# OSU-Nowlab/MPI4DL

Measured on NVIDIA B200. Metric: images/sec (device-timed, max over ranks) AmoebaNet-D 8192^2 hot path (spatial-stage conv/pool fwd+bwd), higher is better.
Workload: dtype bf16

## Files before the change

mpi4dl_b200/csrc/conv_tap.cu:

```cuda
#include <stdlib.h>

#include "common.cuh"
#include "tc_common.cuh"

namespace spc {

using namespace tc;

int make_tmap_ex(CUtensorMap* m, const void* base, int rank, const uint64_t* dims, const uint64_t* strides_bytes,
                 const uint32_t* box, int swizzle128);
int tc_sm_count();

namespace {

constexpr int TAP_THREADS = 448;
constexpr int BLK = 8192;
constexpr int RAW_SHIFT_ROW = 160;
constexpr int MAXRING = 8;
constexpr int STAGE_BYTES = 128 * 128;

struct TapParams {
  int M, Cin, H, W, N;
  int R, ph;
  int Mpad;
  int mrows;
  int a_blk;
  int kchunks;
  int cbox;
  int raw_blk;
  int tiles_w, tiles_h, num_tiles;
  int a_resident, ast, ops;
  int rawb;
  int opblk;
  int group;
  int rows_raw;
  int dbg;
  const __nv_bfloat16* bias;
  __nv_bfloat16* y;
};

struct RingState {
  int s = 0, ph = 0;
  __device__ __forceinline__ void next(int n) { if (++s == n) { s = 0; ph ^= 1; } }
};

template <int D>
__device__ __forceinline__ uint4 shift_window(const uint32_t (&w)[8]) {
  static_assert(D >= -4 && D <= 4, "shift range");
  constexpr int e0 = 4 + D;
  constexpr int k = e0 >> 1;
  uint4 o;
  if (e0 & 1) {
    o.x = __funnelshift_r(w[k], w[k + 1], 16);
    o.y = __funnelshift_r(w[k + 1], w[k + 2], 16);
    o.z = __funnelshift_r(w[k + 2], w[k + 3], 16);
    o.w = __funnelshift_r(w[k + 3], w[k + 4], 16);
  } else {
    o.x = w[k]; o.y = w[k + 1]; o.z = w[k + 2]; o.w = w[k + 3];
  }
  return o;
}

constexpr int SHIFT_THREADS = 256;

template <int NB, int S, int SI>
struct ShiftRow {
  static __device__ __forceinline__ void stores(const uint32_t (&win)[2 * NB][8], int cv, int tid, uint8_t* op_base, int opblk,
                                                int group, uint64_t* op_full, uint64_t* op_empty, RingState& ro, int ops) {
    if constexpr (SI < S) {
      const int q = tid & 7, c0 = tid >> 3;
      const int tile_bytes = NB * opblk;
      if (!group || SI == 0) mbar_wait(&op_empty[ro.s], ro.ph ^ 1);
      uint8_t* opb = op_base + ro.s * (group ? S : 1) * tile_bytes + (group ? SI * tile_bytes : 0);
#pragma unroll
      for (int i = 0; i < 2 * NB; ++i) {
        const int j = i >> 1, c = c0 + 32 * (i & 1);
        if (c < cv)
          *reinterpret_cast<uint4*>(opb + j * opblk + c * 128 + ((q ^ (c & 7)) << 4)) = shift_window<SI - S / 2>(win[i]);
      }
      if (!group || SI == S - 1) {
        fence_proxy_async();
        mbar_arrive(&op_full[ro.s]);
        ro.next(ops);
      }
      ShiftRow<NB, S, SI + 1>::stores(win, cv, tid, op_base, opblk, group, op_full, op_empty, ro, ops);
    }
  }
  static __device__ __forceinline__ void run(const uint8_t* rawr, int raw_blk, int cv, int tid, uint8_t* op_base, int opblk,
                                             int group, uint64_t* op_full, uint64_t* op_empty, RingState& ro, int ops) {
    static_assert(S / 2 <= 4, "filter width <= 9");
    const int q = tid & 7, c0 = tid >> 3;
    uint32_t win[2 * NB][8];
#pragma unroll
    for (int i = 0; i < 2 * NB; ++i) {
      const int j = i >> 1, c = c0 + 32 * (i & 1);
      if (c < cv) {
        const uint8_t* row = rawr + j * raw_blk + c * RAW_SHIFT_ROW;
        const uint4 own = *reinterpret_cast<const uint4*>(row + 16 * (q + 1));
        uint32_t lz = __shfl_up_sync(0xffffffffu, own.z, 1), lw = __shfl_up_sync(0xffffffffu, own.w, 1);
        uint32_t rx = __shfl_down_sync(0xffffffffu, own.x, 1), ry = __shfl_down_sync(0xffffffffu, own.y, 1);
        if (q == 0) { const uint2 h = *reinterpret_cast<const uint2*>(row + 8); lz = h.x; lw = h.y; }
        if (q == 7) { const uint2 h = *reinterpret_cast<const uint2*>(row + 16 * 9); rx = h.x; ry = h.y; }
        win[i][0] = lz; win[i][1] = lw; win[i][2] = own.x; win[i][3] = own.y;
        win[i][4] = own.z; win[i][5] = own.w; win[i][6] = rx; win[i][7] = ry;
      }
    }
    stores(win, cv, tid, op_base, opblk, group, op_full, op_empty, ro, ops);
  }
};

template <int NB, int S>
__global__ void __launch_bounds__(TAP_THREADS, 1)
conv_tap_kernel(const __grid_constant__ CUtensorMap tmap_w, const __grid_constant__ CUtensorMap tmap_x,
                const __grid_constant__ CUtensorMap tmap_y, const TapParams p) {
  constexpr bool SHIFT = S > 1;
  constexpr int NPIX = NB * 64;
  const int RAW_BLK = p.raw_blk;
  extern __shared__ uint8_t smem_raw[];
  uint8_t* smem = reinterpret_cast<uint8_t*>((reinterpret_cast<uintptr_t>(smem_raw) + 1023) & ~(uintptr_t)1023);
  const int taps = p.R * S;
  const int a_blocks = p.a_resident ? taps * p.kchunks : p.ast;
  uint8_t* a_base = smem;
  uint8_t* raw_base = a_base + a_blocks * p.a_blk;
  uint8_t* op_base = raw_base + p.rawb * p.rows_raw * RAW_BLK;
  const int slot_bytes = (p.group ? S : 1) * NB * p.opblk;
  uint8_t* stage_base = op_base + (SHIFT ? p.ops * slot_bytes : 0);
  uint8_t* bar_base = stage_base + STAGE_BYTES;
  uint64_t* raw_full = reinterpret_cast<uint64_t*>(bar_base);
  uint64_t* raw_empty = raw_full + MAXRING;
  uint64_t* a_full = raw_empty + MAXRING;
  uint64_t* a_empty = a_full + MAXRING;
  uint64_t* op_full = a_empty + MAXRING;
  uint64_t* op_empty = op_full + MAXRING;
  uint64_t* tfull = op_empty + MAXRING;
  uint64_t* tempty = tfull + 2;
  uint64_t* a_res_full = tempty + 2;
  uint32_t* tmem_slot = reinterpret_cast<uint32_t*>(a_res_full + 1);

  const int warp = threadIdx.x >> 5, lane = threadIdx.x & 31;

  if (threadIdx.x == 0) {
    for (int i = 0; i < 2; ++i) {
      mbar_init(&tfull[i], 1);
      mbar_init(&tempty[i], 128);
    }
    for (int i = 0; i < MAXRING; ++i) {
      mbar_init(&raw_full[i], 1);
      mbar_init(&raw_empty[i], SHIFT ? SHIFT_THREADS : 1);
      mbar_init(&a_full[i], 1); mbar_init(&a_empty[i], 1);
      mbar_init(&op_full[i], SHIFT_THREADS); mbar_init(&op_empty[i], 1);
    }
    mbar_init(a_res_full, 1);
    fence_barrier_init();
  }
  if (warp == 1) tmem_alloc(tmem_slot, 512);
  tc_fence_before();
  __syncthreads();
  tc_fence_after();
  const uint32_t tmem_base = *tmem_slot;

#define TAP_TILE_DECODE(t)                                        \
  const int tw_ = (t) % p.tiles_w;                                \
  const int th_ = ((t) / p.tiles_w) % p.tiles_h;                  \
  const int n_ = (t) / (p.tiles_w * p.tiles_h);                   \
  const int w0 = tw_ * 64, h0 = th_ * NB;

  if (warp == 0) {
    if (lane == 0) {
      tma_prefetch_desc(&tmap_x);
      tma_prefetch_desc(&tmap_w);
      if (p.a_resident) {
        mbar_arrive_expect_tx(a_res_full, taps * p.kchunks * p.mrows * 128);
        for (int tap = 0; tap < taps; ++tap)
          for (int kc = 0; kc < p.kchunks; ++kc)
            tma_load_2d(a_base + (tap * p.kchunks + kc) * p.a_blk, &tmap_w, a_res_full, kc * 64, tap * p.Mpad);
      }
      RingState rb, ra;
      const int xoff = SHIFT ? 8 : 0;
      int ct = blockIdx.x, ckc = 0;
      const bool noa = p.dbg & 1, noraw = p.dbg & 2;
      if (ct < p.num_tiles && !noraw) {
        TAP_TILE_DECODE(ct)
        mbar_wait(&raw_empty[rb.s], rb.ph ^ 1);
        mbar_arrive_expect_tx(&raw_full[rb.s], p.rows_raw * RAW_BLK);
        for (int i = 0; i < p.rows_raw; ++i)
          tma_load_4d(raw_base + (rb.s * p.rows_raw + i) * RAW_BLK, &tmap_x, &raw_full[rb.s], w0 - xoff, h0 - p.ph + i, 0, n_);
        rb.next(p.rawb);
      }
      while (ct < p.num_tiles) {
        int nt = ct, nkc = ckc + 1;
        if (nkc == p.kchunks) { nkc = 0; nt = ct + gridDim.x; }
        const bool has_next = nt < p.num_tiles && !noraw;
        TAP_TILE_DECODE(has_next ? nt : ct)
        uint8_t* dst = raw_base + rb.s * p.rows_raw * RAW_BLK;
        bool armed = false;
        int row = 0;
        for (int tap = 0; tap < taps; ++tap) {
          if (!p.a_resident && !noa) {
            mbar_wait(&a_empty[ra.s], ra.ph ^ 1);
            mbar_arrive_expect_tx(&a_full[ra.s], p.mrows * 128);
            tma_load_2d(a_base + ra.s * p.a_blk, &tmap_w, &a_full[ra.s], ckc * 64, tap * p.Mpad);
            ra.next(p.ast);
          }
          if (has_next) {
            if (!armed && mbar_test_wait(&raw_empty[rb.s], rb.ph ^ 1)) {
              mbar_arrive_expect_tx(&raw_full[rb.s], p.rows_raw * RAW_BLK);
              armed = true;
            }
            if (armed) {
              const int quota = ((tap + 1) * p.rows_raw + taps - 1) / taps;
              for (; row < quota; ++row)
                tma_load_4d(dst + row * RAW_BLK, &tmap_x, &raw_full[rb.s], w0 - xoff, h0 - p.ph + row, nkc * 64, n_);
            }
          }
        }
        if (has_next) {
          if (!armed) {
            mbar_wait(&raw_empty[rb.s], rb.ph ^ 1);
            mbar_arrive_expect_tx(&raw_full[rb.s], p.rows_raw * RAW_BLK);
          }
          for (; row < p.rows_raw; ++row)
            tma_load_4d(dst + row * RAW_BLK, &tmap_x, &raw_full[rb.s], w0 - xoff, h0 - p.ph + row, nkc * 64, n_);
          rb.next(p.rawb);
        }
        ct = nt; ckc = nkc;
      }
    }
  } else if (warp == 1) {
    if (lane == 0) {
      constexpr uint32_t IDESC = umma_idesc_bf16(128, NPIX, 0, 1);
      if (p.a_resident) { mbar_wait(a_res_full, 0); tc_fence_after(); }
      RingState rb, ra, ro;
      int acc = 0, aph = 0;
      for (int t = blockIdx.x; t < p.num_tiles; t += gridDim.x) {
        mbar_wait(&tempty[acc], aph ^ 1);
        tc_fence_after();
        for (int kc = 0; kc < p.kchunks; ++kc) {
          if (!SHIFT && !(p.dbg & 2)) { mbar_wait(&raw_full[rb.s], rb.ph); tc_fence_after(); }
          const int nsteps = min(4, (p.Cin - kc * 64 + 15) / 16);
          for (int tap = 0; tap < taps; ++tap) {
            uint32_t sb;
            const int si = tap % S;
            if (SHIFT) {
              if (!p.group || si == 0) mbar_wait(&op_full[ro.s], ro.ph);
              sb = smem_u32(op_base + ro.s * slot_bytes + (p.group ? si * NB * p.opblk : 0));
            } else {
              sb = smem_u32(raw_base + (rb.s * p.rows_raw + tap) * RAW_BLK);
            }
            uint32_t sa;
            if (p.a_resident) {
              sa = smem_u32(a_base + (tap * p.kchunks + kc) * p.a_blk);
            } else {
              if (!(p.dbg & 1)) mbar_wait(&a_full[ra.s], ra.ph);
              sa = smem_u32(a_base + ra.s * p.a_blk);
            }
            tc_fence_after();
            for (int ks = 0; ks < nsteps; ++ks) {
              const uint64_t bdesc = umma_desc(sb + ks * 2048, SHIFT ? p.opblk : RAW_BLK, 1024);
              const uint64_t adesc = umma_desc(sa + ks * 32, 16, 1024);
              umma_bf16(tmem_base + acc * NPIX, adesc, bdesc, IDESC, (kc | tap | ks) ? 1u : 0u);
            }
            if (SHIFT && (!p.group || si == S - 1)) { umma_commit(&op_empty[ro.s]); ro.next(p.ops); }
            if (!p.a_resident) { if (!(p.dbg & 1)) umma_commit(&a_empty[ra.s]); ra.next(p.ast); }
          }
          if (!SHIFT) { if (!(p.dbg & 2)) umma_commit(&raw_empty[rb.s]); rb.next(p.rawb); }
        }
        umma_commit(&tfull[acc]);
        if (++acc == 2) { acc = 0; aph ^= 1; }
      }
    }
  } else if (warp >= 6) {
    if (SHIFT) {
      const int tid = threadIdx.x - 6 * 32;
      RingState rb, ro;
      for (int t = blockIdx.x; t < p.num_tiles; t += gridDim.x) {
        for (int kc = 0; kc < p.kchunks; ++kc) {
          if (!(p.dbg & 2)) mbar_wait(&raw_full[rb.s], rb.ph);
          const int cv = (p.dbg & 8) ? 0 : min(64, (p.Cin - kc * 64 + 15) & ~15);
          const uint8_t* rawb = raw_base + rb.s * p.rows_raw * RAW_BLK;
          for (int r = 0; r < p.R; ++r)
            ShiftRow<NB, S, 0>::run(rawb + r * RAW_BLK, RAW_BLK, cv, tid, op_base, p.opblk, p.group, op_full, op_empty, ro, p.ops);
          if (!(p.dbg & 2)) mbar_arrive(&raw_empty[rb.s]);
          rb.next(p.rawb);
        }
      }
    }
  } else if (warp >= 2 && warp <= 5) {
    const int quarter = warp & 3;
    const int k = quarter * 32 + lane;
    const float bias = (k < p.M && p.bias) ? __bfloat162float(p.bias[k]) : 0.f;
    const bool leader = threadIdx.x == 64;
    int acc = 0, aph = 0;
    for (int t = blockIdx.x; t < p.num_tiles; t += gridDim.x) {
      TAP_TILE_DECODE(t)
      mbar_wait(&tfull[acc], aph);
      tc_fence_after();
#pragma unroll 1
      for (int j = 0; j < NB; ++j) {
        if (leader) tma_store_wait_read<0>();
        named_bar_sync(1, 128);
#pragma unroll
        for (int cc = 0; cc < 2; ++cc) {
          uint32_t r[32];
          tmem_ld_32x32(tmem_base + ((uint32_t)(quarter * 32) << 16) + acc * NPIX + j * 64 + cc * 32, r);
          tmem_ld_wait();
          uint8_t* rowp = stage_base + k * 128;
#pragma unroll
          for (int v = 0; v < 4; ++v) {
            uint4 o;
            o.x = pack_bf16x2(__uint_as_float(r[8 * v + 0]) + bias, __uint_as_float(r[8 * v + 1]) + bias);
            o.y = pack_bf16x2(__uint_as_float(r[8 * v + 2]) + bias, __uint_as_float(r[8 * v + 3]) + bias);
            o.z = pack_bf16x2(__uint_as_float(r[8 * v + 4]) + bias, __uint_as_float(r[8 * v + 5]) + bias);
            o.w = pack_bf16x2(__uint_as_float(r[8 * v + 6]) + bias, __uint_as_float(r[8 * v + 7]) + bias);
            const int chunk = (cc * 4 + v) ^ (k & 7);
            *reinterpret_cast<uint4*>(rowp + chunk * 16) = o;
          }
        }
        if (j == NB - 1) {
          tc_fence_before();
          mbar_arrive(&tempty[acc]);
        }
        fence_proxy_async();
        named_bar_sync(1, 128);
        if (leader && !(p.dbg & 4) && h0 + j < p.H) {
          tma_store_4d(&tmap_y, stage_base, w0, h0 + j, 0, n_);
          tma_store_commit();
        }
      }
      if (++acc == 2) { acc = 0; aph ^= 1; }
    }
    if (leader) tma_store_wait_read<0>();
  }
#undef TAP_TILE_DECODE
  tc_fence_before();
  __syncthreads();
  if (warp == 1) tmem_dealloc(tmem_base, 512);
}

constexpr int TAP_SMEM_LIMIT = 222 * 1024;
constexpr int TAP_SMEM_AUX = 1024  + 1024 ;

inline int round_up_i(int a, int b) { return (a + b - 1) / b * b; }

struct TapPlan {
  int NB;
  TapParams p;
  int smem;
};

bool plan_tap(int M, int Cin, int R, int S, int H, int W, int N, TapPlan* out) {
  TapParams p{};
  p.M = M; p.Cin = Cin; p.H = H; p.W = W; p.N = N; p.R = R;
  p.mrows = round_up_i(M, 8);
  p.a_blk = round_up_i(p.mrows * 128, 1024);
  p.kchunks = (Cin + 63) / 64;
  const int taps = R * S;
  const bool shift = S > 1;
  p.cbox = Cin >= 64 ? 64 : round_up_i(Cin, 16);
  p.raw_blk = p.cbox * (shift ? RAW_SHIFT_ROW : 128);
  const int raw_blk = p.raw_blk;
  const int budget = TAP_SMEM_LIMIT - TAP_SMEM_AUX;
  p.opblk = p.cbox * 128;
  const int budget_ops = budget - STAGE_BYTES;
  for (int NB = 4; NB >= 2; NB -= 2) {
    if (NB == 4 && H < 4) continue;
    p.rows_raw = NB + R - 1;
    const int raw_buf = p.rows_raw * raw_blk;
    const int a_res = taps * p.kchunks * p.a_blk;
    for (int resident = 1; resident >= 0; --resident) {
      for (int group = shift ? 1 : 0; group >= 0; --group) {
        const int slot = (group ? S : 1) * NB * p.opblk;
        int ast = resident ? 0 : 3;
        int a_bytes = resident ? a_res : ast * p.a_blk;
        int rawb = 2, ops = shift ? 2 : 0;
        int rem = budget_ops - a_bytes - rawb * raw_buf - ops * slot;
        if (rem < 0) continue;
        if (shift && !group && rem >= slot) { ++ops; rem -= slot; }
        while (!resident && ast < MAXRING && rem >= p.a_blk) { ++ast; rem -= p.a_blk; }
        while (rawb < 4 && rem >= raw_buf) { ++rawb; rem -= raw_buf; }
        while (shift && ops < 4 && rem >= slot) { ++ops; rem -= slot; }
        a_bytes = resident ? a_res : ast * p.a_blk;
        p.a_resident = resident; p.ast = ast; p.ops = ops; p.rawb = rawb; p.group = group;
        out->NB = NB; out->p = p;
        out->smem = a_bytes + rawb * raw_buf + ops * slot + STAGE_BYTES + TAP_SMEM_AUX;
        return true;
      }
    }
  }
  return false;
}

template <int NB, int S>
int launch_tap(const CUtensorMap& tw, const CUtensorMap& tx, const CUtensorMap& ty, const TapParams& p, int smem,
               cudaStream_t st) {
  auto kern = conv_tap_kernel<NB, S>;
  static bool attr_set = false;
  if (!attr_set) {
    SPC_CHECK_CUDA(cudaFuncSetAttribute(kern, cudaFuncAttributeMaxDynamicSharedMemorySize, TAP_SMEM_LIMIT));
    attr_set = true;
  }
  const int sms = tc_sm_count();
  const int grid = p.num_tiles < sms ? p.num_tiles : sms;
  kern<<<grid, TAP_THREADS, smem, st>>>(tw, tx, ty, p);
  count_launch();
  SPC_CHECK_CUDA(cudaGetLastError());
  return SPC_OK;
}

}

bool tap_v2_supported(int M, int Cin, int R, int S, int H, int W, int N, int stride) {
  if (stride != 1 || M > 128 || R * S == 1 || (W % 64) != 0 || H < 2) return false;
  if (!(S == 1 || S == 3 || S == 5 || S == 7) || (R & 1) == 0 || R > 7) return false;
  TapPlan pl;
  return plan_tap(M, Cin, R, S, H, W, N, &pl);
}

int run_conv_tap_v2(const __nv_bfloat16* wp, int Mpad, int Cpad, const __nv_bfloat16* x, const __nv_bfloat16* bias,
                    __nv_bfloat16* y, int M, int Cin, int R, int S, int ph, int H, int W, int N, cudaStream_t st) {
  TapPlan pl;
  SPC_REQUIRE(plan_tap(M, Cin, R, S, H, W, N, &pl), "tap conv: no shared-memory plan for M=%d Cin=%d %dx%d", M, Cin, R, S);
  TapParams& p = pl.p;
  p.ph = ph; p.Mpad = Mpad; p.bias = bias; p.y = y;
  {
    const char* e = getenv("SPC_TAP_DBG");
    p.dbg = e ? atoi(e) : 0;
  }
  p.tiles_w = W / 64;
  p.tiles_h = (H + pl.NB - 1) / pl.NB;
  p.num_tiles = p.tiles_w * p.tiles_h * N;
  CUtensorMap tw, tx, ty;
  {
    const uint64_t dims[2] = {(uint64_t)Cpad, (uint64_t)R * S * Mpad};
    const uint64_t strides[2] = {0, (uint64_t)Cpad * 2};
    const uint32_t box[2] = {64, (uint32_t)p.mrows};
    int rc = make_tmap_ex(&tw, wp, 2, dims, strides, box, 1);
    if (rc) return rc;
  }
  {
    const uint64_t dims[4] = {(uint64_t)W, (uint64_t)H, (uint64_t)Cin, (uint64_t)N};
    const uint64_t strides[4] = {0, (uint64_t)W * 2, (uint64_t)H * W * 2, (uint64_t)H * W * Cin * 2};
    const uint32_t box[4] = {(uint32_t)(S > 1 ? 80 : 64), 1, (uint32_t)p.cbox, 1};
    int rc = make_tmap_ex(&tx, x, 4, dims, strides, box, S > 1 ? 0 : 1);
    if (rc) return rc;
  }
  {
    const uint64_t dims[4] = {(uint64_t)W, (uint64_t)H, (uint64_t)M, (uint64_t)N};
    const uint64_t strides[4] = {0, (uint64_t)W * 2, (uint64_t)H * W * 2, (uint64_t)H * W * M * 2};
    const uint32_t box[4] = {64, 1, 128, 1};
    int rc = make_tmap_ex(&ty, y, 4, dims, strides, box, 1);
    if (rc) return rc;
  }
#define TAP_CASE(nb, s) if (pl.NB == nb && S == s) return launch_tap<nb, s>(tw, tx, ty, p, pl.smem, st);
  TAP_CASE(2, 1) TAP_CASE(4, 1) TAP_CASE(2, 3) TAP_CASE(4, 3) TAP_CASE(2, 5) TAP_CASE(4, 5) TAP_CASE(2, 7) TAP_CASE(4, 7)
#undef TAP_CASE
  set_error("tap conv: unsupported filter width %d", S);
  return SPC_EUNSUPPORTED;
}

}
```

mpi4dl_b200/csrc/gemm_tc.cu:

```cuda
#include <stdlib.h>

#include "common.cuh"
#include "tc_common.cuh"

namespace spc {

using namespace tc;

bool tap_v2_supported(int M, int Cin, int R, int S, int H, int W, int N, int stride);
int run_conv_tap_v2(const __nv_bfloat16* wp, int Mpad, int Cpad, const __nv_bfloat16* x, const __nv_bfloat16* bias,
                    __nv_bfloat16* y, int M, int Cin, int R, int S, int ph, int H, int W, int N, cudaStream_t st);

bool wgrad_tap_supported(int K, int C, int R, int S, int H, int W, int stride);
int run_wgrad_tap(const __nv_bfloat16* x, const __nv_bfloat16* dy, float* dw, int K, int C, int N, int H, int W, int R, int S,
                  cudaStream_t st);

namespace {

constexpr int TC_THREADS = 192;
constexpr int BK = 64;
constexpr int A_BLK_BYTES = 128 * BK * 2;
constexpr int B_BLK_BYTES = BK * 64 * 2;
constexpr int TMEM_COLS = 512;

typedef CUresult (*EncodeTiledFn)(CUtensorMap*, CUtensorMapDataType, cuuint32_t, void*, const cuuint64_t*,
                                  const cuuint64_t*, const cuuint32_t*, const cuuint32_t*, CUtensorMapInterleave,
                                  CUtensorMapSwizzle, CUtensorMapL2promotion, CUtensorMapFloatOOBfill);
EncodeTiledFn get_encode() {
  static EncodeTiledFn fn = nullptr;
  if (!fn) {
    void* p = nullptr;
    cudaDriverEntryPointQueryResult q;
    if (cudaGetDriverEntryPoint("cuTensorMapEncodeTiled", &p, cudaEnableDefault, &q) == cudaSuccess &&
        q == cudaDriverEntryPointSuccess)
      fn = reinterpret_cast<EncodeTiledFn>(p);
  }
  return fn;
}

int make_tmap_sw(CUtensorMap* m, const void* base, int rank, const uint64_t* dims, const uint64_t* strides_bytes,
                 const uint32_t* box, CUtensorMapSwizzle swz) {
  EncodeTiledFn enc = get_encode();
  if (!enc) {
    set_error("cuTensorMapEncodeTiled entry point not available");
    return SPC_ECUDA;
  }
  static thread_local bool ctx_bound = false;
  if (!ctx_bound) {
    if (cudaFree(nullptr) != cudaSuccess) {
      set_error("tcgen05 conv: no CUDA context on this thread");
      return SPC_ECUDA;
    }
    ctx_bound = true;
  }
  cuuint64_t gd[5], gs[5];
  cuuint32_t bx[5], es[5];
  for (int i = 0; i < rank; ++i) {
    gd[i] = dims[i];
    bx[i] = box[i];
    es[i] = 1;
    if (i > 0) gs[i - 1] = strides_bytes[i];
  }
  CUresult r = enc(m, CU_TENSOR_MAP_DATA_TYPE_BFLOAT16, (cuuint32_t)rank, const_cast<void*>(base), gd, gs, bx, es,
                   CU_TENSOR_MAP_INTERLEAVE_NONE, swz, CU_TENSOR_MAP_L2_PROMOTION_L2_256B,
                   CU_TENSOR_MAP_FLOAT_OOB_FILL_NONE);
  if (r != CUDA_SUCCESS) {
    set_error("cuTensorMapEncodeTiled failed (%d) rank=%d dims=[%llu,%llu,%llu] strides=[%llu,%llu]", (int)r, rank,
              (unsigned long long)dims[0], (unsigned long long)(rank > 1 ? dims[1] : 0),
              (unsigned long long)(rank > 2 ? dims[2] : 0), (unsigned long long)(rank > 1 ? strides_bytes[1] : 0),
              (unsigned long long)(rank > 2 ? strides_bytes[2] : 0));
    return SPC_ECUDA;
  }
  return SPC_OK;
}

int make_tmap(CUtensorMap* m, const void* base, int rank, const uint64_t* dims, const uint64_t* strides_bytes,
              const uint32_t* box) {
  return make_tmap_sw(m, base, rank, dims, strides_bytes, box, CU_TENSOR_MAP_SWIZZLE_128B);
}

__global__ void repack_weights_kernel(const __nv_bfloat16* __restrict__ w, __nv_bfloat16* __restrict__ wp, int M,
                                      int Cc, int Mpad, int Cpad, int taps, long long sm, long long sc, int flip) {
  const int total = taps * Mpad * Cpad;
  for (int i = blockIdx.x * blockDim.x + threadIdx.x; i < total; i += gridDim.x * blockDim.x) {
    const int c = i % Cpad;
    const int m = (i / Cpad) % Mpad;
    const int tap = i / (Cpad * Mpad);
    __nv_bfloat16 v = __float2bfloat16(0.f);
    if (m < M && c < Cc) v = w[(size_t)m * sm + (size_t)c * sc + (flip ? taps - 1 - tap : tap)];
    wp[i] = v;
  }
}

constexpr int BN_DEFAULT = 128;
constexpr int OUT_BUF_BYTES = 128 * 128 * 2;
constexpr int MAX_STAGES = 8;

struct PwParams {
  int M;
  int Cin;
  int P;
  int N;
  int tiles_per_image;
  int num_mg;
  int num_tiles;
  int stages;
  int wres;
  int out_bufs;
  int taps, S, ph, pw;
  int W, Mpad;
  int shiftN;
  int rowmul;
  int tgroup;
  const __nv_bfloat16* bias;
  __nv_bfloat16* y;
  int epi_stg;
  int x5, y5;
  int stationary_ok;
  int xbox, ybox;
};

template <int MB, int BN, bool EXT>
__global__ void __launch_bounds__(TC_THREADS, 1)
pw_gemm_kernel(const __grid_constant__ CUtensorMap tmap_w, const __grid_constant__ CUtensorMap tmap_x,
               const __grid_constant__ CUtensorMap tmap_x4, const __grid_constant__ CUtensorMap tmap_y,
               const PwParams p) {
  constexpr int NB = BN / 64;
  constexpr int ACC = (MB <= 2) ? 2 : 1;
  static_assert(ACC * MB * BN <= TMEM_COLS, "TMEM budget");
  extern __shared__ uint8_t smem_raw[];
  uint8_t* smem = reinterpret_cast<uint8_t*>((reinterpret_cast<uintptr_t>(smem_raw) + 1023) & ~(uintptr_t)1023);
  const int kchunks = (p.Cin + BK - 1) / BK;
  const int ksteps_total = (p.Cin + 15) / 16;
  const int iters = p.taps * kchunks;
  const int wres_bytes = p.wres ? iters * MB * A_BLK_BYTES : 0;
  const int stage_bytes = (p.wres ? 0 : MB * A_BLK_BYTES) + NB * B_BLK_BYTES;
  uint8_t* wres = smem;
  uint8_t* stage0 = smem + wres_bytes;
  uint8_t* outbuf = stage0 + p.stages * stage_bytes;
  uint64_t* full = reinterpret_cast<uint64_t*>(outbuf + p.out_bufs * OUT_BUF_BYTES);
  uint64_t* empty = full + MAX_STAGES;
  uint64_t* tfull = empty + MAX_STAGES;
  uint64_t* tempty = tfull + 2;
  uint64_t* wfull = tempty + 2;
  uint32_t* tmem_slot = reinterpret_cast<uint32_t*>(wfull + 1);

  const int warp = threadIdx.x >> 5, lane = threadIdx.x & 31;
  const bool x5 = EXT && p.x5, y5 = EXT && p.y5, epi_stg = EXT && p.epi_stg;
  const int xbox = EXT ? p.xbox : BK, ybox = EXT ? p.ybox : 128;

  if (threadIdx.x == 0) {
    for (int i = 0; i < p.stages; ++i) { mbar_init(&full[i], 1); mbar_init(&empty[i], 1); }
    for (int i = 0; i < ACC; ++i) { mbar_init(&tfull[i], 1); mbar_init(&tempty[i], 128); }
    mbar_init(wfull, 1);
    fence_barrier_init();
  }
  if (warp == 1) tmem_alloc(tmem_slot, TMEM_COLS);
  tc_fence_before();
  __syncthreads();
  tc_fence_after();
  const uint32_t tmem_base = *tmem_slot;

  if (warp == 0) {
    if (lane == 0) {
      tma_prefetch_desc(&tmap_w);
      tma_prefetch_desc(&tmap_x);
      if (p.wres) {
        const int mg0 = blockIdx.x % p.num_mg;
        mbar_arrive_expect_tx(wfull, wres_bytes);
        for (int it = 0; it < iters; ++it)
#pragma unroll
          for (int mb = 0; mb < MB; ++mb)
            tma_load_2d(wres + (it * MB + mb) * A_BLK_BYTES, &tmap_w, wfull, (it % kchunks) * BK,
                        (it / kchunks) * p.Mpad + mg0 * (MB * 128) + mb * 128);
      }
      int s = 0, ph = 0;
      for (int it = 0;; ++it) {
        const int t = ((it / p.tgroup) * gridDim.x + blockIdx.x) * p.tgroup + it % p.tgroup;
        if ((it / p.tgroup) * gridDim.x * p.tgroup >= p.num_tiles) break;
        if (t >= p.num_tiles) continue;
        const int mg = t % p.num_mg;
        const int tt = t / p.num_mg;
        const int n = tt / p.tiles_per_image;
        const int p0 = (tt % p.tiles_per_image) * BN;
        for (int it = 0; it < iters; ++it) {
          const int kc = it % kchunks, tap = it / kchunks;
          mbar_wait(&empty[s], ph ^ 1);
          uint8_t* st = stage0 + s * stage_bytes;
          mbar_arrive_expect_tx(&full[s], stage_bytes);
          if (!p.wres) {
#pragma unroll
            for (int mb = 0; mb < MB; ++mb)
              tma_load_2d(st + mb * A_BLK_BYTES, &tmap_w, &full[s], kc * BK, tap * p.Mpad + mg * (MB * 128) + mb * 128);
            st += MB * A_BLK_BYTES;
          }
          if (p.taps == 1) {
            if (x5) {
              tma_load_5d(st, &tmap_x, &full[s], 0, 0, p0 >> 6, kc * (BK / 8), n);
            } else if (xbox == BK) {
#pragma unroll
              for (int j = 0; j < NB; ++j) tma_load_3d(st + j * B_BLK_BYTES, &tmap_x, &full[s], p0 + j * 64, kc * BK, n);
            } else {
              for (int cg = 0; cg < BK; cg += xbox)
#pragma unroll
                for (int j = 0; j < NB; ++j)
                  tma_load_3d(st + j * B_BLK_BYTES + cg * 128, &tmap_x, &full[s], p0 + j * 64, kc * BK + cg, n);
            }
          } else {
            const int dr = tap / p.S - p.ph;
            const int img = n + (tap % p.S) * p.shiftN;
#pragma unroll
            for (int j = 0; j < NB; ++j) {
              const int q = p0 + j * 64, hq = q / p.W, wq = q - hq * p.W;
              tma_load_4d(st + j * B_BLK_BYTES, &tmap_x4, &full[s], wq, hq * p.rowmul + dr, kc * BK, img);
            }
          }
          if (++s == p.stages) { s = 0; ph ^= 1; }
        }
      }
    }
  } else if (warp == 1) {
    if (lane == 0) {
      constexpr uint32_t IDESC = umma_idesc_bf16(128, BN, 0, 1);
      if (p.wres) { mbar_wait(wfull, 0); tc_fence_after(); }
      int s = 0, ph = 0, a = 0, aph = 0;
      for (int it = 0;; ++it) {
        const int t = ((it / p.tgroup) * gridDim.x + blockIdx.x) * p.tgroup + it % p.tgroup;
        if ((it / p.tgroup) * gridDim.x * p.tgroup >= p.num_tiles) break;
        if (t >= p.num_tiles) continue;
        mbar_wait(&tempty[a], aph ^ 1);
        tc_fence_after();
        for (int it = 0; it < iters; ++it) {
          const int kc = it % kchunks;
          mbar_wait(&full[s], ph);
          tc_fence_after();
          const uint32_t st = smem_u32(stage0 + s * stage_bytes);
          const uint32_t sa = p.wres ? smem_u32(wres + it * MB * A_BLK_BYTES) : st;
          const uint32_t sb = p.wres ? st : st + MB * A_BLK_BYTES;
          const int nsteps = min(4, ksteps_total - kc * 4);
          for (int ks = 0; ks < nsteps; ++ks) {
            const uint64_t bdesc = x5 ? umma_desc(sb + ks * (NB * 2048), 1024, NB * 1024)
                                        : umma_desc(sb + ks * 2048, B_BLK_BYTES, 1024);
#pragma unroll
            for (int mb = 0; mb < MB; ++mb) {
              const uint64_t adesc = umma_desc(sa + mb * A_BLK_BYTES + ks * 32, 16, 1024);
              umma_bf16(tmem_base + (a * MB + mb) * BN, adesc, bdesc, IDESC, (it | ks) ? 1u : 0u);
            }
          }
          umma_commit(&empty[s]);
          if (it == iters - 1) umma_commit(&tfull[a]);
          if (++s == p.stages) { s = 0; ph ^= 1; }
        }
        if (++a == ACC) { a = 0; aph ^= 1; }
      }
    }
  } else {
    const int quarter = warp & 3;
    const int row = quarter * 32 + lane;
    const bool leader = (threadIdx.x == 64);
    int a = 0, aph = 0, ob = 0;
    for (int it = 0;; ++it) {
      const int t = ((it / p.tgroup) * gridDim.x + blockIdx.x) * p.tgroup + it % p.tgroup;
      if ((it / p.tgroup) * gridDim.x * p.tgroup >= p.num_tiles) break;
      if (t >= p.num_tiles) continue;
      const int mg = t % p.num_mg;
      const int tt = t / p.num_mg;
      const int n = tt / p.tiles_per_image;
      const int p0 = (tt % p.tiles_per_image) * BN;
      mbar_wait(&tfull[a], aph);
      tc_fence_after();
#pragma unroll 1
      for (int mb = 0; mb < MB; ++mb) {
        const int k0 = mg * (MB * 128) + mb * 128;
        if (k0 >= p.M) break;
        const int k = k0 + row;
        const float bias = (k < p.M && p.bias) ? __bfloat162float(p.bias[k]) : 0.f;
#pragma unroll 1
        for (int h = 0; h < BN / 128; ++h) {
          const int ph0 = p0 + h * 128;
          uint8_t* buf = outbuf + ob * OUT_BUF_BYTES;
          if (epi_stg) {
            if (p.out_bufs == 1) named_bar_sync(1, 128);
          } else {
            if (leader) { if (p.out_bufs == 2) tma_store_wait_read<1>(); else tma_store_wait_read<0>(); }
            named_bar_sync(1, 128);
          }
#pragma unroll
          for (int cc = 0; cc < 4; ++cc) {
            uint32_t r[32];
            tmem_ld_32x32(tmem_base + ((uint32_t)(quarter * 32) << 16) + (a * MB + mb) * BN + h * 128 + cc * 32, r);
            tmem_ld_wait();
            uint8_t* blk = y5 ? buf + (row >> 3) * 2048 + (cc >> 1) * 1024 + (row & 7) * 128
                                : buf + (cc >> 1) * (128 * 128) + row * 128;
#pragma unroll
            for (int q = 0; q < 4; ++q) {
              uint4 v;
              v.x = pack_bf16x2(__uint_as_float(r[8 * q + 0]) + bias, __uint_as_float(r[8 * q + 1]) + bias);
              v.y = pack_bf16x2(__uint_as_float(r[8 * q + 2]) + bias, __uint_as_float(r[8 * q + 3]) + bias);
              v.z = pack_bf16x2(__uint_as_float(r[8 * q + 4]) + bias, __uint_as_float(r[8 * q + 5]) + bias);
              v.w = pack_bf16x2(__uint_as_float(r[8 * q + 6]) + bias, __uint_as_float(r[8 * q + 7]) + bias);
              const int chunk = ((cc & 1) * 4 + q) ^ (row & 7);
              *reinterpret_cast<uint4*>(blk + chunk * 16) = v;
            }
          }
          if (h == BN / 128 - 1 && (mb == MB - 1 || k0 + 128 >= p.M)) {
            tc_fence_before();
            mbar_arrive(&tempty[a]);
          }
          if (epi_stg) {
            named_bar_sync(1, 128);
            const int et = threadIdx.x - 64, g = et & 7, r0 = et >> 3;
#pragma unroll
            for (int j = 0; j < 2; ++j) {
              const int px = ph0 + j * 64 + g * 8;
              if (px < p.P) {
#pragma unroll
                for (int rr = 0; rr < 8; ++rr) {
                  const int rw = rr * 16 + r0;
                  if (k0 + rw < p.M) {
                    const uint4 v = *reinterpret_cast<const uint4*>(buf + j * (128 * 128) + rw * 128 + ((g ^ (rw & 7)) << 4));
                    __stcs(reinterpret_cast<uint4*>(p.y + ((size_t)n * p.M + k0 + rw) * p.P + px), v);
                  }
                }
              }
            }
          } else {
            fence_proxy_async();
            named_bar_sync(1, 128);
            if (leader) {
              if (y5) {
                tma_store_5d(&tmap_y, buf, 0, 0, ph0 >> 6, k0 >> 3, n);
              } else if (ybox == 128) {
#pragma unroll
                for (int j = 0; j < 2; ++j) tma_store_3d(&tmap_y, buf + j * (128 * 128), ph0 + j * 64, k0, n);
              } else {
                for (int cg = 0; cg < 128 && k0 + cg < p.M; cg += ybox)
#pragma unroll
                  for (int j = 0; j < 2; ++j)
                    tma_store_3d(&tmap_y, buf + j * (128 * 128) + cg * 128, ph0 + j * 64, k0 + cg, n);
              }
              tma_store_commit();
            }
          }
          if (p.out_bufs == 2) ob ^= 1;
        }
      }
      if (++a == ACC) { a = 0; aph ^= 1; }
    }
    if (leader && !epi_stg) tma_store_wait_read<0>();
  }

  tc_fence_before();
  __syncthreads();
  if (warp == 1) tmem_dealloc(tmem_base, TMEM_COLS);
}

inline int round_up(int a, int b) { return (a + b - 1) / b * b; }
struct EnvKnob { const char* name; const char* val; };
EnvKnob g_env_tab[32];
int g_env_n = 0;
inline const char* env_get(const char* name) {
  for (int i = 0; i < g_env_n; ++i)
    if (g_env_tab[i].name == name) return g_env_tab[i].val;
  const char* v = getenv(name);
  if (g_env_n < 32) { g_env_tab[g_env_n].name = name; g_env_tab[g_env_n].val = v; ++g_env_n; }
  return v;
}
inline int env_int(const char* name, int dflt) {
  const char* e = env_get(name);
  const int v = e ? atoi(e) : 0;
  return v > 0 ? v : dflt;
}
inline int sm_count() {
  static int sms = 0;
  if (!sms) {
    int dev = 0;
    cudaGetDevice(&dev);
    if (cudaDeviceGetAttribute(&sms, cudaDevAttrMultiProcessorCount, dev) != cudaSuccess || sms <= 0) sms = 148;
  }
  return sms;
}

constexpr int SMEM_LIMIT = 222 * 1024;
constexpr int SMEM_AUX = 1024  + 512 ;

template <int MB, int BN, bool EXT>
int launch_pw_ext(const CUtensorMap& tw, const CUtensorMap& tx, const CUtensorMap& tx4, const CUtensorMap& ty, PwParams p,
              cudaStream_t st) {
  const int kchunks = (p.Cin + BK - 1) / BK;
  const int budget = SMEM_LIMIT - SMEM_AUX;
  const int wres_bytes = p.taps * kchunks * MB * A_BLK_BYTES;
  const int sms = sm_count();
  int grid = p.num_tiles < sms ? p.num_tiles : sms;
  if (p.num_tiles < 16 * sms) p.tgroup = 1;
  bool stationary = wres_bytes <= 128 * 1024;
  if (stationary && p.num_mg > 1) {
    if (p.stationary_ok && grid >= 4 * p.num_mg) { grid = grid / p.num_mg * p.num_mg; p.tgroup = 1; }
    else stationary = false;
  }
  p.wres = stationary ? 1 : 0;
  const int stage_bytes = (p.wres ? 0 : MB * A_BLK_BYTES) + (BN / 64) * B_BLK_BYTES;
  const int rem = budget - (p.wres ? wres_bytes : 0);
  p.out_bufs = 2;
  p.stages = (rem - 2 * OUT_BUF_BYTES) / stage_bytes;
  if (p.stages < 3 || env_int("SPC_PW_OUTBUFS", 2) == 1) { p.out_bufs = 1; p.stages = (rem - OUT_BUF_BYTES) / stage_bytes; }
  if (p.stages > MAX_STAGES) p.stages = MAX_STAGES;
  SPC_REQUIRE(p.stages >= 2, "tcgen05 conv: shared memory budget too small (MB=%d kchunks=%d)", MB, kchunks);
  const int smem = (p.wres ? wres_bytes : 0) + p.stages * stage_bytes + p.out_bufs * OUT_BUF_BYTES + SMEM_AUX;
  auto kern = pw_gemm_kernel<MB, BN, EXT>;
  static bool attr_set = false;
  if (!attr_set) {
    SPC_CHECK_CUDA(cudaFuncSetAttribute(kern, cudaFuncAttributeMaxDynamicSharedMemorySize, SMEM_LIMIT));
    attr_set = true;
  }
  kern<<<grid, TC_THREADS, smem, st>>>(tw, tx, tx4, ty, p);
  count_launch();
  SPC_CHECK_CUDA(cudaGetLastError());
  return SPC_OK;
}

template <int MB, int BN>
int launch_pw(const CUtensorMap& tw, const CUtensorMap& tx, const CUtensorMap& tx4, const CUtensorMap& ty, const PwParams& p,
              cudaStream_t st) {
  const bool ext = p.x5 || p.y5 || p.epi_stg || p.xbox != BK || p.ybox != 128;
  return ext ? launch_pw_ext<MB, BN, true>(tw, tx, tx4, ty, p, st) : launch_pw_ext<MB, BN, false>(tw, tx, tx4, ty, p, st);
}

int make_act_tmap(CUtensorMap* m, const void* base, int P, int Cc, int N, int box_rows) {
  const uint64_t dims[3] = {(uint64_t)P, (uint64_t)Cc, (uint64_t)N};
  const uint64_t strides[3] = {0, (uint64_t)P * 2, (uint64_t)P * Cc * 2};
  const uint32_t box[3] = {64, (uint32_t)box_rows, 1};
  return make_tmap(m, base, 3, dims, strides, box);
}

int make_act_tmap5(CUtensorMap* m, const void* base, int P, int Cc, int N, int groups, int blocks) {
  const uint64_t dims[5] = {64, 8, (uint64_t)P / 64, (uint64_t)Cc / 8, (uint64_t)N};
  const uint64_t strides[5] = {0, (uint64_t)P * 2, 128, (uint64_t)P * 16, (uint64_t)P * Cc * 2};
  const uint32_t box[5] = {64, 8, (uint32_t)blocks, (uint32_t)groups, 1};
  return make_tmap(m, base, 5, dims, strides, box);
}

int launch_shift_copies(const void* x, void* xs, size_t planes, int H, int W, int S, int pw, int cs, cudaStream_t st);

struct TcConv {
  const __nv_bfloat16* w;
  long long sm, sc;
  int flip;
  int M, Cin;
  int R, S, ph, pw;
  int H, W, N;
  int stride;
  const __nv_bfloat16* prepacked;
};

int run_conv_tc(const TcConv& c, const __nv_bfloat16* x, const __nv_bfloat16* bias, __nv_bfloat16* y, void* ws,
                size_t ws_bytes, cudaStream_t st) {
  const int taps = c.R * c.S;
  const int cs = c.stride;
  const int Ho = c.H / cs, Wo = c.W / cs;
  const int Pin = c.H * c.W, P = Ho * Wo;
  const int Mpad = round_up(c.M, 128), Cpad = round_up(c.Cin, BK);
  const bool v2 = taps > 1 && !env_get("SPC_TAP_V1") && tap_v2_supported(c.M, c.Cin, c.R, c.S, c.H, c.W, c.N, cs);
  const bool copies = (c.S > 1 || cs > 1) && taps > 1 && !v2;
  const uintptr_t ws0 = reinterpret_cast<uintptr_t>(ws);
  const uintptr_t wp_addr = (ws0 + 1023) & ~(uintptr_t)1023;
  const size_t wp_bytes = c.prepacked ? 0 : (size_t)taps * Mpad * Cpad * 2;
  const uintptr_t xs_addr = (wp_addr + wp_bytes + 1023) & ~(uintptr_t)1023;
  const size_t xs_bytes = copies ? (size_t)c.S * c.N * c.Cin * c.H * Wo * 2 : 0;
  const size_t need = (xs_addr - ws0) + xs_bytes;
  SPC_REQUIRE((ws && ws_bytes >= need) || need <= 1024, "tcgen05 conv: workspace too small (%zu < %zu)", ws_bytes, need);
  const __nv_bfloat16* wp = c.prepacked;
  if (!c.prepacked) {
    __nv_bfloat16* wpm = reinterpret_cast<__nv_bfloat16*>(wp_addr);
    const int total = taps * Mpad * Cpad;
    int blocks = (total + 255) / 256;
    if (blocks > 1184) blocks = 1184;
    repack_weights_kernel<<<blocks, 256, 0, st>>>(c.w, wpm, c.M, c.Cin, Mpad, Cpad, taps, c.sm, c.sc, c.flip);
    count_launch();
    SPC_CHECK_CUDA(cudaGetLastError());
    wp = wpm;
  }
  if (v2)
    return run_conv_tap_v2(wp, Mpad, Cpad, x, bias, y, c.M, c.Cin, c.R, c.S, c.ph, c.H, c.W, c.N, st);
  const __nv_bfloat16* xsrc = x;
  if (copies) {
    void* xs = reinterpret_cast<void*>(xs_addr);
    int rc0 = launch_shift_copies(x, xs, (size_t)c.N * c.Cin, c.H, c.W, c.S, c.pw, cs, st);
    if (rc0) return rc0;
    xsrc = reinterpret_cast<const __nv_bfloat16*>(xs);
  }
  CUtensorMap tw, tx, tx4, ty;
  const char* n256_env = env_get("SPC_PW_N256");
  const bool n256 = taps == 1 && cs == 1 && Mpad / 128 >= 3 && (Cpad / BK) * A_BLK_BYTES <= 128 * 1024 && P % 256 == 0 &&
                    (n256_env ? atoi(n256_env) != 0 : false);
  const int BN = n256 ? 256 : BN_DEFAULT;
  int xbox = (taps == 1) ? env_int("SPC_PW_XBOX", BK) : BK, ybox = env_int("SPC_PW_YBOX", 128);
  if (xbox != 8 && xbox != 16 && xbox != 32) xbox = BK;
  if (ybox != 8 && ybox != 16 && ybox != 32 && ybox != 64) ybox = 128;
  const char* box5_env = env_get("SPC_PW_BOX5");
  const int box5 = box5_env ? atoi(box5_env) : ((size_t)P * 2 >= ((size_t)4 << 20) ? 3 : 0);
  const int x5 = (taps == 1 && cs == 1 && (box5 & 1) && P % 64 == 0 && c.Cin % 8 == 0 && xbox == BK) ? 1 : 0;
  const int y5 = (taps == 1 && (box5 & 2) && P % 64 == 0 && c.M % 8 == 0 && ybox == 128) ? 1 : 0;
  {
    const uint64_t dims[2] = {(uint64_t)Cpad, (uint64_t)taps * Mpad};
    const uint64_t strides[2] = {0, (uint64_t)Cpad * 2};
    const uint32_t box[2] = {BK, 128};
    int rc = make_tmap(&tw, wp, 2, dims, strides, box);
    if (rc) return rc;
  }
  int rc;
  if (taps > 1) {
    const uint64_t dims[4] = {(uint64_t)Wo, (uint64_t)c.H, (uint64_t)c.Cin, (uint64_t)c.N * (copies ? c.S : 1)};
    const uint64_t strides[4] = {0, (uint64_t)Wo * 2, (uint64_t)c.H * Wo * 2, (uint64_t)c.H * Wo * c.Cin * 2};
    const uint32_t box[4] = {64, 1, BK, 1};
    rc = make_tmap(&tx4, xsrc, 4, dims, strides, box);
    if (rc) return rc;
    tx = tx4;
  } else {
    rc = x5 ? make_act_tmap5(&tx, x, Pin, c.Cin, c.N, BK / 8, BN / 64) : make_act_tmap(&tx, x, Pin, c.Cin, c.N, xbox);
    if (rc) return rc;
    tx4 = tx;
  }
  rc = y5 ? make_act_tmap5(&ty, y, P, c.M, c.N, 16, 2) : make_act_tmap(&ty, y, P, c.M, c.N, ybox);
  if (rc) return rc;
  PwParams p{};
  p.xbox = xbox; p.ybox = ybox; p.x5 = x5; p.y5 = y5;
  p.bias = bias; p.M = c.M; p.Cin = c.Cin; p.P = P; p.N = c.N;
  p.taps = taps; p.S = c.S; p.ph = c.ph; p.pw = c.pw; p.W = Wo; p.Mpad = Mpad;
  p.shiftN = copies ? c.N : 0;
  p.rowmul = cs;
  p.y = y;
  p.epi_stg = (env_int("SPC_PW_EPI_STG", 0) == 1 && P % 8 == 0 && !y5) ? 1 : 0;
  {
    const char* e = env_get("SPC_TILE_GROUP");
    p.tgroup = e ? atoi(e) : 1;
    if (p.tgroup < 1) p.tgroup = 1;
  }
  const int MBtot = Mpad / 128;
  int mb = MBtot >= 3 ? (c.Cin <= 512 ? 2 : 4) : MBtot;
  {
    const char* se = env_get("SPC_PW_STATIONARY");
    const int kch = (c.Cin + BK - 1) / BK;
    p.stationary_ok = ((se && atoi(se) != 0) || n256) && taps * kch * A_BLK_BYTES <= 128 * 1024;
    if (p.stationary_ok && MBtot >= 3 && !n256) mb = (taps * kch * 2 * A_BLK_BYTES <= 128 * 1024) ? 2 : 1;
    if (n256) mb = 1;
  }
  if (MBtot >= 3 && !n256 && env_get("SPC_PW_MB4")) mb = 4;
  if (MBtot >= 3 && !n256 && env_get("SPC_PW_MB2")) mb = 2;
  p.num_mg = (MBtot + mb - 1) / mb;
  p.tiles_per_image = (P + BN - 1) / BN;
  p.num_tiles = p.tiles_per_image * c.N * p.num_mg;
  if (n256) return launch_pw<1, 256>(tw, tx, tx4, ty, p, st);
  if (mb == 1) return launch_pw<1, 128>(tw, tx, tx4, ty, p, st);
  if (mb == 2) return launch_pw<2, 128>(tw, tx, tx4, ty, p, st);
  return launch_pw<4, 128>(tw, tx, tx4, ty, p, st);
}

int run_pw(const __nv_bfloat16* w, int ld, int transpose, int M, int Cin, const __nv_bfloat16* x,
           const __nv_bfloat16* bias, __nv_bfloat16* y, int N, int P, void* ws, size_t ws_bytes, cudaStream_t st) {
  TcConv c{};
  c.w = w;
  c.sm = transpose ? 1 : ld; c.sc = transpose ? ld : 1; c.flip = 0;
  c.M = M; c.Cin = Cin; c.R = 1; c.S = 1; c.ph = 0; c.pw = 0; c.H = 1; c.W = P; c.N = N; c.stride = 1;
  return run_conv_tc(c, x, bias, y, ws, ws_bytes, st);
}

struct WgParams {
  float* dw;
  int K, C, P, N;
  int nblk;
  int n_blocks;
  int mgroups;
  int splits;
  int chunks_total;
  int chunks_per_image;
  int stages;
  int taps, S, ph;
  int TG, passes;
  int W, shiftN;
  int rowmul;
  int mrows;
  int split_major;
  int pb;
  int dy5, x5;
};

template <int MG>
__global__ void __launch_bounds__(TC_THREADS, 1)
pw_wgrad_kernel(const __grid_constant__ CUtensorMap tmap_dy, const __grid_constant__ CUtensorMap tmap_x,
                const __grid_constant__ CUtensorMap tmap_x4, const WgParams p) {
  extern __shared__ uint8_t smem_raw[];
  uint8_t* smem = reinterpret_cast<uint8_t*>((reinterpret_cast<uintptr_t>(smem_raw) + 1023) & ~(uintptr_t)1023);
  const int b_bytes = p.nblk * 128;
  const int b_slot = (b_bytes + 1023) & ~1023;
  const int stage_bytes = p.pb * (MG * A_BLK_BYTES + p.TG * b_slot);
  uint64_t* full = reinterpret_cast<uint64_t*>(smem + p.stages * stage_bytes);
  uint64_t* empty = full + MAX_STAGES;
  uint64_t* tfull = empty + MAX_STAGES;
  uint64_t* tempty = tfull + 1;
  uint32_t* tmem_slot = reinterpret_cast<uint32_t*>(tempty + 1);
  const int warp = threadIdx.x >> 5, lane = threadIdx.x & 31;

  if (threadIdx.x == 0) {
    for (int i = 0; i < p.stages; ++i) { mbar_init(&full[i], 1); mbar_init(&empty[i], 1); }
    mbar_init(tfull, 1);
    mbar_init(tempty, 128);
    fence_barrier_init();
  }
  if (warp == 1) tmem_alloc(tmem_slot, TMEM_COLS);
  tc_fence_before();
  __syncthreads();
  tc_fence_after();
  const uint32_t tmem_base = *tmem_slot;
  const int ngroups = p.mgroups * p.n_blocks * p.passes;
  const int num_items = ngroups * p.splits;
  const int per_split = (p.chunks_total + p.splits - 1) / p.splits;

#define WG_DECODE(it)                                                        \
  const int sp = p.split_major ? (it) / ngroups : (it) % p.splits;           \
  const int g_ = p.split_major ? (it) % ngroups : (it) / p.splits;           \
  const int pass = g_ % p.passes;                                            \
  const int nb = (g_ / p.passes) % p.n_blocks;                               \
  const int mgp = g_ / (p.passes * p.n_blocks);                              \
  const int tap0 = pass * p.TG;                                              \
  const int ntap = min(p.TG, p.taps - tap0);                                 \
  const int c_begin = sp * per_split, c_end = min(p.chunks_total, c_begin + per_split);

  if (warp == 0) {
    if (lane == 0) {
      tma_prefetch_desc(&tmap_dy);
      tma_prefetch_desc(&tmap_x);
      int s = 0, ph = 0;
      for (int it = blockIdx.x; it < num_items; it += gridDim.x) {
        WG_DECODE(it)
        (void)mgp;
        for (int ch = c_begin; ch < c_end; ++ch) {
          const int n = ch / p.chunks_per_image, p0 = (ch % p.chunks_per_image) * (64 * p.pb);
          mbar_wait(&empty[s], ph ^ 1);
          uint8_t* st = smem + s * stage_bytes;
          mbar_arrive_expect_tx(&full[s], p.pb * (MG * p.mrows * 128 + ntap * b_bytes));
          if (p.pb == 2) {
#pragma unroll
            for (int i = 0; i < MG; ++i) {
              uint8_t* da = st + i * (2 * A_BLK_BYTES);
              const int r0 = (mgp * MG + i) * p.mrows;
              if (p.dy5) {
                tma_load_5d(da, &tmap_dy, &full[s], 0, 0, p0 >> 6, r0 >> 3, n);
              } else {
                tma_load_3d(da, &tmap_dy, &full[s], p0, r0, n);
                tma_load_3d(da + A_BLK_BYTES, &tmap_dy, &full[s], p0 + 64, r0, n);
              }
            }
            uint8_t* xa = st + MG * (2 * A_BLK_BYTES);
            if (p.x5) {
              tma_load_5d(xa, &tmap_x, &full[s], 0, 0, p0 >> 6, (nb * p.nblk) >> 3, n);
            } else {
              tma_load_3d(xa, &tmap_x, &full[s], p0, nb * p.nblk, n);
              tma_load_3d(xa + b_slot, &tmap_x, &full[s], p0 + 64, nb * p.nblk, n);
            }
            if (++s == p.stages) { s = 0; ph ^= 1; }
            continue;
          }
#pragma unroll
          for (int i = 0; i < MG; ++i)
            tma_load_3d(st + i * A_BLK_BYTES, &tmap_dy, &full[s], p0, (mgp * MG + i) * p.mrows, n);
          if (p.taps == 1) {
            tma_load_3d(st + MG * A_BLK_BYTES, &tmap_x, &full[s], p0, nb * p.nblk, n);
          } else {
            const int hq = p0 / p.W, wq = p0 - hq * p.W;
            for (int t = 0; t < ntap; ++t) {
              const int tap = tap0 + t;
              tma_load_4d(st + MG * A_BLK_BYTES + t * b_slot, &tmap_x4, &full[s], wq, hq * p.rowmul + tap / p.S - p.ph,
                          nb * p.nblk, n + (tap % p.S) * p.shiftN);
            }
          }
          if (++s == p.stages) { s = 0; ph ^= 1; }
        }
      }
    }
  } else if (warp == 1) {
    if (lane == 0) {
      const uint32_t idesc = umma_idesc_bf16(128, p.nblk, 0, 0);
      int s = 0, ph = 0, aph = 0;
      for (int it = blockIdx.x; it < num_items; it += gridDim.x) {
        WG_DECODE(it)
        (void)nb; (void)mgp;
        mbar_wait(tempty, aph ^ 1);
        tc_fence_after();
        for (int ch = c_begin; ch < c_end; ++ch) {
          mbar_wait(&full[s], ph);
          tc_fence_after();
          const uint32_t sa = smem_u32(smem + s * stage_bytes);
          if (p.pb == 2) {
            const uint32_t sb = sa + MG * (2 * A_BLK_BYTES);
            const uint32_t aj = p.dy5 ? 1024 : A_BLK_BYTES, asbo = p.dy5 ? 2048 : 1024;
            const uint32_t bj = p.x5 ? 1024 : b_slot, bsbo = p.x5 ? 2048 : 1024;
#pragma unroll
            for (int j = 0; j < 2; ++j) {
#pragma unroll
              for (int ks = 0; ks < 4; ++ks) {
                const uint64_t bdesc = umma_desc(sb + j * bj + ks * 32, 16, bsbo);
#pragma unroll
                for (int i = 0; i < MG; ++i) {
                  const uint64_t adesc = umma_desc(sa + i * (2 * A_BLK_BYTES) + j * aj + ks * 32, 16, asbo);
                  umma_bf16(tmem_base + i * p.nblk, adesc, bdesc, idesc, (ch > c_begin || ks > 0 || j > 0) ? 1u : 0u);
                }
              }
            }
            umma_commit(&empty[s]);
            if (++s == p.stages) { s = 0; ph ^= 1; }
            continue;
          }
          const uint32_t sb = sa + MG * A_BLK_BYTES;
          for (int t = 0; t < ntap; ++t) {
#pragma unroll
            for (int ks = 0; ks < 4; ++ks) {
              const uint64_t bdesc = umma_desc(sb + t * b_slot + ks * 32, 16, 1024);
#pragma unroll
              for (int i = 0; i < MG; ++i) {
                const uint64_t adesc = umma_desc(sa + i * A_BLK_BYTES + ks * 32, 16, 1024);
                umma_bf16(tmem_base + (t * MG + i) * p.nblk, adesc, bdesc, idesc, (ch > c_begin || ks > 0) ? 1u : 0u);
              }
            }
          }
          umma_commit(&empty[s]);
          if (++s == p.stages) { s = 0; ph ^= 1; }
        }
        umma_commit(tfull);
        aph ^= 1;
      }
    }
  } else {
    const int quarter = warp & 3;
    int aph = 0;
    for (int it = blockIdx.x; it < num_items; it += gridDim.x) {
      WG_DECODE(it)
      mbar_wait(tfull, aph);
      tc_fence_after();
      if (c_end > c_begin) {
#pragma unroll 1
        for (int t = 0; t < ntap; ++t) {
#pragma unroll 1
          for (int i = 0; i < MG; ++i) {
            const int rib = quarter * 32 + lane;
            const int k = rib < p.mrows ? (mgp * MG + i) * p.mrows + rib : p.K;
#pragma unroll 1
            for (int cc = 0; cc * 32 < p.nblk; ++cc) {
              uint32_t r[32];
              tmem_ld_32x32(tmem_base + ((uint32_t)(quarter * 32) << 16) + (t * MG + i) * p.nblk + cc * 32, r);
              tmem_ld_wait();
              if (k < p.K) {
#pragma unroll
                for (int j = 0; j < 32; ++j) {
                  const int cl = cc * 32 + j;
                  const int c = nb * p.nblk + cl;
                  if (cl < p.nblk && c < p.C)
                    atomicAdd(&p.dw[((size_t)k * p.C + c) * p.taps + tap0 + t], __uint_as_float(r[j]));
                }
              }
            }
          }
        }
      }
      tc_fence_before();
      mbar_arrive(tempty);
      aph ^= 1;
    }
  }
#undef WG_DECODE
  tc_fence_before();
  __syncthreads();
  if (warp == 1) tmem_dealloc(tmem_base, TMEM_COLS);
}

template <int MG>
int launch_wg(const CUtensorMap& tdy, const CUtensorMap& tx, const CUtensorMap& tx4, WgParams p, cudaStream_t st) {
  const int b_slot = (p.nblk * 128 + 1023) & ~1023;
  int TG = 512 / (MG * p.nblk);
  if (TG > p.taps) TG = p.taps;
  while (TG > 1 && MG * A_BLK_BYTES + TG * b_slot > (SMEM_LIMIT - SMEM_AUX) / 2) --TG;
  p.TG = TG;
  p.passes = (p.taps + TG - 1) / TG;
  const int stage_bytes = p.pb * (MG * A_BLK_BYTES + TG * b_slot);
  p.stages = (SMEM_LIMIT - SMEM_AUX) / stage_bytes;
  if (p.stages > 6) p.stages = 6;
  p.stages = min(p.stages, env_int("SPC_WG_STAGES", p.stages));
  SPC_REQUIRE(p.stages >= 2, "tcgen05 wgrad: smem budget");
  const int sms = sm_count();
  const int groups = p.mgroups * p.n_blocks * p.passes;
  int splits = 1;
  {
    const double clk = 1.8e9;
    const double bytes_chunk = (double)p.pb * (MG * p.mrows + p.TG * p.nblk) * 128.0;
    const double mma_chunk = (double)p.pb * MG * p.TG * 4.0 * (p.nblk > 64 ? p.nblk : 64) / 256.0 * 222.0;
    const double t_chunk = (bytes_chunk / 40.0 > mma_chunk ? bytes_chunk / 40.0 : mma_chunk) / clk;
    const double elems = (double)MG * p.mrows * p.nblk * p.TG;
    const int smax = (2 * sms) / groups > 1 ? (2 * sms) / groups : 1;
    double best = 1e30;
    for (int s = smax; s >= 1; --s) {
      if (s > p.chunks_total / 8 && s > 1) continue;
      const int items_s = groups * s, waves = (items_s + sms - 1) / sms;
      const double cpi = (double)((p.chunks_total + s - 1) / s);
      const double t = waves * cpi * t_chunk + (double)items_s * elems / 90e9;
      if (t < best * 0.98) { best = t; splits = s; }
    }
  }
  if (env_get("SPC_WG_SPLIT_CEIL")) splits = (2 * sms + groups - 1) / groups;
  splits = env_int("SPC_WG_SPLITS", splits);
  if (splits > p.chunks_total / 8) splits = p.chunks_total / 8;
  if (splits < 1) splits = 1;
  p.splits = splits;
  p.split_major = env_get("SPC_WG_GROUP_MAJOR") ? 0 : 1;
  const int smem = p.stages * stage_bytes + SMEM_AUX;
  auto kern = pw_wgrad_kernel<MG>;
  static bool attr_set = false;
  if (!attr_set) {
    SPC_CHECK_CUDA(cudaFuncSetAttribute(kern, cudaFuncAttributeMaxDynamicSharedMemorySize, SMEM_LIMIT));
    attr_set = true;
  }
  const int items = groups * p.splits;
  kern<<<items < sms ? items : sms, TC_THREADS, smem, st>>>(tdy, tx, tx4, p);
  count_launch();
  SPC_CHECK_CUDA(cudaGetLastError());
  return SPC_OK;
}

template <int MP>
__global__ void __cluster_dims__(2, 1, 1) __launch_bounds__(TC_THREADS, 1)
pw_wgrad_pair_kernel(const __grid_constant__ CUtensorMap tmap_dy, const __grid_constant__ CUtensorMap tmap_x,
                     const WgParams p) {
  extern __shared__ uint8_t smem_raw[];
  uint8_t* smem = reinterpret_cast<uint8_t*>((reinterpret_cast<uintptr_t>(smem_raw) + 1023) & ~(uintptr_t)1023);
  const int half = p.nblk / 2;
  const int b_bytes = half * 128;
  const int b_slot = (b_bytes + 1023) & ~1023;
  const int stage_bytes = p.pb * (MP * A_BLK_BYTES + b_slot);
  uint64_t* full = reinterpret_cast<uint64_t*>(smem + p.stages * stage_bytes);
  uint64_t* empty = full + MAX_STAGES;
  uint64_t* tfull = empty + MAX_STAGES;
  uint64_t* tempty = tfull + 1;
  uint32_t* tmem_slot = reinterpret_cast<uint32_t*>(tempty + 1);
  const int warp = threadIdx.x >> 5, lane = threadIdx.x & 31;
  const uint32_t rank = cluster_ctarank();
  const int cluster_id = blockIdx.x >> 1, num_clusters = gridDim.x >> 1;

  if (threadIdx.x == 0) {
    for (int i = 0; i < p.stages; ++i) { mbar_init(&full[i], 2); mbar_init(&empty[i], 1); }
    mbar_init(tfull, 1);
    mbar_init(tempty, 256);
    fence_barrier_init();
  }
  if (warp == 1) tmem_alloc_2sm(tmem_slot, TMEM_COLS);
  tc_fence_before();
  cluster_sync_all();
  tc_fence_after();
  const uint32_t tmem_base = *tmem_slot;
  const int ngroups = p.mgroups * p.n_blocks;
  const int num_items = ngroups * p.splits;
  const int per_split = (p.chunks_total + p.splits - 1) / p.splits;
  const uint32_t stage_tx = 2u * (uint32_t)p.pb * (uint32_t)(MP * p.mrows * 128 + b_bytes);

#define WGP_DECODE(it)                                                          \
  const int sp = (it) / ngroups;                                               \
  const int g_ = (it) % ngroups;                                               \
  const int nb = g_ % p.n_blocks;                                              \
  const int mgp = g_ / p.n_blocks;                                             \
  const int c_begin = sp * per_split, c_end = min(p.chunks_total, c_begin + per_split);

  if (warp == 0) {
    if (lane == 0) {
      tma_prefetch_desc(&tmap_dy);
      tma_prefetch_desc(&tmap_x);
      int s = 0, ph = 0;
      for (int it = cluster_id; it < num_items; it += num_clusters) {
        WGP_DECODE(it)
        for (int ch = c_begin; ch < c_end; ++ch) {
          const int n = ch / p.chunks_per_image, p0 = (ch % p.chunks_per_image) * (64 * p.pb);
          mbar_wait(&empty[s], ph ^ 1);
          uint8_t* st = smem + s * stage_bytes;
          if (rank == 0) mbar_arrive_expect_tx(&full[s], stage_tx);
          else mbar_arrive_cluster(&full[s], 0);
          if (p.pb == 2) {
#pragma unroll
            for (int i = 0; i < MP; ++i)
              tma_load_5d_2sm(st + i * (2 * A_BLK_BYTES), &tmap_dy, &full[s], 0, 0, p0 >> 6,
                              (((mgp * MP + i) * 2 + (int)rank) * p.mrows) >> 3, n);
            tma_load_5d_2sm(st + MP * (2 * A_BLK_BYTES), &tmap_x, &full[s], 0, 0, p0 >> 6,
                            (nb * p.nblk + (int)rank * half) >> 3, n);
            if (++s == p.stages) { s = 0; ph ^= 1; }
            continue;
          }
#pragma unroll
          for (int i = 0; i < MP; ++i)
            tma_load_3d_2sm(st + i * A_BLK_BYTES, &tmap_dy, &full[s], p0, ((mgp * MP + i) * 2 + (int)rank) * p.mrows, n);
          tma_load_3d_2sm(st + MP * A_BLK_BYTES, &tmap_x, &full[s], p0, nb * p.nblk + (int)rank * half, n);
          if (++s == p.stages) { s = 0; ph ^= 1; }
        }
      }
    }
  } else if (warp == 1) {
    if (lane == 0 && rank == 0) {
      const uint32_t idesc = umma_idesc_bf16(256, p.nblk, 0, 0);
      int s = 0, ph = 0, aph = 0;
      for (int it = cluster_id; it < num_items; it += num_clusters) {
        WGP_DECODE(it)
        (void)nb; (void)mgp;
        mbar_wait(tempty, aph ^ 1);
        tc_fence_after();
        for (int ch = c_begin; ch < c_end; ++ch) {
          mbar_wait(&full[s], ph);
          tc_fence_after();
          const uint32_t sa = smem_u32(smem + s * stage_bytes);
          if (p.pb == 2) {
            const uint32_t sb = sa + MP * (2 * A_BLK_BYTES);
#pragma unroll
            for (int j = 0; j < 2; ++j) {
#pragma unroll
              for (int ks = 0; ks < 4; ++ks) {
                const uint64_t bdesc = umma_desc(sb + j * 1024 + ks * 32, 16, 2048);
#pragma unroll
                for (int i = 0; i < MP; ++i) {
                  const uint64_t adesc = umma_desc(sa + i * (2 * A_BLK_BYTES) + j * 1024 + ks * 32, 16, 2048);
                  umma_bf16_2sm(tmem_base + i * p.nblk, adesc, bdesc, idesc, (ch > c_begin || ks > 0 || j > 0) ? 1u : 0u);
                }
              }
            }
            umma_commit_2sm(&empty[s]);
            if (++s == p.stages) { s = 0; ph ^= 1; }
            continue;
          }
          const uint32_t sb = sa + MP * A_BLK_BYTES;
#pragma unroll
          for (int ks = 0; ks < 4; ++ks) {
            const uint64_t bdesc = umma_desc(sb + ks * 32, 16, 1024);
#pragma unroll
            for (int i = 0; i < MP; ++i) {
              const uint64_t adesc = umma_desc(sa + i * A_BLK_BYTES + ks * 32, 16, 1024);
              umma_bf16_2sm(tmem_base + i * p.nblk, adesc, bdesc, idesc, (ch > c_begin || ks > 0) ? 1u : 0u);
            }
          }
          umma_commit_2sm(&empty[s]);
          if (++s == p.stages) { s = 0; ph ^= 1; }
        }
        umma_commit_2sm(tfull);
        aph ^= 1;
      }
    }
  } else {
    const int quarter = warp & 3;
    int aph = 0;
    for (int it = cluster_id; it < num_items; it += num_clusters) {
      WGP_DECODE(it)
      mbar_wait(tfull, aph);
      tc_fence_after();
      if (c_end > c_begin) {
#pragma unroll 1
        for (int i = 0; i < MP; ++i) {
          const int rib = quarter * 32 + lane;
          const int k = rib < p.mrows ? ((mgp * MP + i) * 2 + (int)rank) * p.mrows + rib : p.K;
#pragma unroll 1
          for (int cc = 0; cc * 32 < p.nblk; ++cc) {
            uint32_t r[32];
            tmem_ld_32x32(tmem_base + ((uint32_t)(quarter * 32) << 16) + i * p.nblk + cc * 32, r);
            tmem_ld_wait();
            if (k < p.K) {
#pragma unroll
              for (int j = 0; j < 32; ++j) {
                const int cl = cc * 32 + j;
                const int c = nb * p.nblk + cl;
                if (cl < p.nblk && c < p.C) atomicAdd(&p.dw[(size_t)k * p.C + c], __uint_as_float(r[j]));
              }
            }
          }
        }
      }
      tc_fence_before();
      mbar_arrive_cluster(tempty, 0);
      aph ^= 1;
    }
  }
#undef WGP_DECODE
  tc_fence_before();
  cluster_sync_all();
  if (warp == 1) tmem_dealloc_2sm(tmem_base, TMEM_COLS);
}

template <int MP>
int launch_wg_pair(const CUtensorMap& tdy, const CUtensorMap& tx, WgParams p, cudaStream_t st) {
  const int b_slot = ((p.nblk / 2) * 128 + 1023) & ~1023;
  const int stage_bytes = p.pb * (MP * A_BLK_BYTES + b_slot);
  p.stages = (SMEM_LIMIT - SMEM_AUX) / stage_bytes;
  if (p.stages > 6) p.stages = 6;
  p.stages = min(p.stages, env_int("SPC_WG_STAGES", p.stages));
  SPC_REQUIRE(p.stages >= 2, "tcgen05 pair wgrad: smem budget");
  const int sms = sm_count();
  const int clusters = sms / 2;
  const int groups = p.mgroups * p.n_blocks;
  int splits = 1;
  {
    const double clk = 1.8e9;
    const double bytes_chunk = (double)p.pb * (MP * p.mrows + p.nblk / 2) * 128.0;
    const double mma_chunk = (double)p.pb * MP * 4.0 * (p.nblk > 64 ? p.nblk : 64) / 256.0 * 222.0;
    const double t_chunk = (bytes_chunk / 40.0 > mma_chunk ? bytes_chunk / 40.0 : mma_chunk) / clk;
    const double elems = 2.0 * MP * p.mrows * p.nblk;
    const int smax = (2 * clusters) / groups > 1 ? (2 * clusters) / groups : 1;
    double best = 1e30;
    for (int s = smax; s >= 1; --s) {
      if (s > p.chunks_total / 8 && s > 1) continue;
      const int items_s = groups * s, waves = (items_s + clusters - 1) / clusters;
      const double cpi = (double)((p.chunks_total + s - 1) / s);
      const double t = waves * cpi * t_chunk + (double)items_s * elems / 90e9;
      if (t < best * 0.98) { best = t; splits = s; }
    }
  }
  splits = env_int("SPC_WG_SPLITS", splits);
  if (splits > p.chunks_total / 8) splits = p.chunks_total / 8;
  if (splits < 1) splits = 1;
  p.splits = splits;
  const int smem = p.stages * stage_bytes + SMEM_AUX;
  auto kern = pw_wgrad_pair_kernel<MP>;
  static bool attr_set = false;
  if (!attr_set) {
    SPC_CHECK_CUDA(cudaFuncSetAttribute(kern, cudaFuncAttributeMaxDynamicSharedMemorySize, SMEM_LIMIT));
    attr_set = true;
  }
  const int items = groups * p.splits;
  const int grid = 2 * (items < clusters ? items : clusters);
  kern<<<grid, TC_THREADS, smem, st>>>(tdy, tx, p);
  count_launch();
  SPC_CHECK_CUDA(cudaGetLastError());
  return SPC_OK;
}

int run_wgrad(const __nv_bfloat16* x, const __nv_bfloat16* dy, float* dw, int K, int C, int N, int Ho, int Wo, int Hin,
              int R, int S, int ph, int stride, bool copies, cudaStream_t st) {
  const int P = Ho * Wo;
  WgParams p{};
  p.dw = dw; p.K = K; p.C = C; p.P = P; p.N = N;
  p.taps = R * S; p.S = S; p.ph = ph; p.W = Wo; p.shiftN = copies ? N : 0; p.rowmul = stride;
  const int nblk_max = min(256, round_up(env_int("SPC_WG_NBLK", 256), 16));
  p.n_blocks = (C + nblk_max - 1) / nblk_max;
  p.nblk = round_up((C + p.n_blocks - 1) / p.n_blocks, 16);
  int MBtot = (K + 127) / 128;
  p.mrows = env_get("SPC_WG_ROWS128") ? 128 : round_up((K + MBtot - 1) / MBtot, 8);
  MBtot = (K + p.mrows - 1) / p.mrows;
  int MG = p.taps > 1 ? 1 : 512 / p.nblk;
  if (MG > MBtot) MG = MBtot;
  MG = min(MG, env_int("SPC_WG_MG", MG));
  MG = MG >= 4 ? 4 : (MG >= 2 ? 2 : 1);
  p.mgroups = (MBtot + MG - 1) / MG;
  p.chunks_per_image = (P + 63) / 64;
  p.chunks_total = p.chunks_per_image * N;
  p.pb = 1;
  const bool pair = p.taps == 1 && (env_get("SPC_WG_2CTA") ? true : (env_get("SPC_WG_1CTA") ? false : C >= 400)) &&
                    MBtot >= 2 && p.nblk % 16 == 0;
  {
    const char* we = env_get("SPC_WG_WIDE");
    const bool wide = p.taps == 1 && !pair && P % 128 == 0 && (we ? atoi(we) != 0 : (size_t)P * 2 >= ((size_t)2 << 20));
    if (wide) {
      const int b_slot = (p.nblk * 128 + 1023) & ~1023;
      while (MG > 1 && 2 * 2 * (MG * A_BLK_BYTES + b_slot) > SMEM_LIMIT - SMEM_AUX) MG >>= 1;
      p.mgroups = (MBtot + MG - 1) / MG;
      p.pb = 2;
      p.chunks_per_image = P / 128;
      p.chunks_total = p.chunks_per_image * N;
      const char* be = env_get("SPC_WG_BOX5");
      const int b5 = be ? atoi(be) : 3;
      p.dy5 = ((b5 & 1) && K % 8 == 0 && p.mrows % 8 == 0) ? 1 : 0;
      p.x5 = ((b5 & 2) && C % 8 == 0 && p.nblk % 8 == 0) ? 1 : 0;
    }
  }
  CUtensorMap tdy, tx, tx4;
  int rc = p.dy5 ? make_act_tmap5(&tdy, dy, P, K, N, p.mrows / 8, 2) : make_act_tmap(&tdy, dy, P, K, N, p.mrows);
  if (rc) return rc;
  if (p.taps > 1) {
    const uint64_t dims[4] = {(uint64_t)Wo, (uint64_t)Hin, (uint64_t)C, (uint64_t)N * (copies ? S : 1)};
    const uint64_t strides[4] = {0, (uint64_t)Wo * 2, (uint64_t)Hin * Wo * 2, (uint64_t)Hin * Wo * C * 2};
    const uint32_t box[4] = {64, 1, (uint32_t)p.nblk, 1};
    rc = make_tmap(&tx4, x, 4, dims, strides, box);
    if (rc) return rc;
    tx = tx4;
  } else {
    rc = p.x5 ? make_act_tmap5(&tx, x, P, C, N, p.nblk / 8, 2) : make_act_tmap(&tx, x, P, C, N, p.nblk);
    if (rc) return rc;
    tx4 = tx;
  }
  if (pair) {
    const int npairs = (MBtot + 1) / 2;
    int MP = 512 / p.nblk;
    if (MP > npairs) MP = npairs;
    MP = MP >= 2 ? 2 : 1;
    CUtensorMap txh;
    const char* we = env_get("SPC_WG_PAIR_WIDE");
    const bool wide = P % 128 == 0 && K % 8 == 0 && C % 8 == 0 && p.mrows % 8 == 0 && p.nblk % 16 == 0 &&
                      (we ? atoi(we) != 0 : (size_t)P * 2 >= ((size_t)2 << 20));
    if (wide) {
      const int b_slot = ((p.nblk / 2) * 128 + 1023) & ~1023;
      if (MP == 2 && env_get("SPC_WG_PAIR_MP1")) MP = 1;
      while (MP > 1 && 2 * 2 * (MP * A_BLK_BYTES + b_slot) > SMEM_LIMIT - SMEM_AUX) MP >>= 1;
      p.pb = 2;
      p.chunks_per_image = P / 128;
      p.chunks_total = p.chunks_per_image * N;
      rc = make_act_tmap5(&tdy, dy, P, K, N, p.mrows / 8, 2);
      if (rc) return rc;
      rc = make_act_tmap5(&txh, x, P, C, N, p.nblk / 16, 2);
    } else {
      rc = make_act_tmap(&txh, x, P, C, N, p.nblk / 2);
    }
    if (rc) return rc;
    p.mgroups = (npairs + MP - 1) / MP;
    return MP == 2 ? launch_wg_pair<2>(tdy, txh, p, st) : launch_wg_pair<1>(tdy, txh, p, st);
  }
  if (MG == 1) return launch_wg<1>(tdy, tx, tx4, p, st);
  if (MG == 2) return launch_wg<2>(tdy, tx, tx4, p, st);
  return launch_wg<4>(tdy, tx, tx4, p, st);
}

__global__ void repack_dgrad_s2_kernel(const __nv_bfloat16* __restrict__ w, __nv_bfloat16* __restrict__ wp, int K,
                                       int C, int Mpad, int Kpad) {
  const int total = 4 * Mpad * Kpad;
  for (int i = blockIdx.x * blockDim.x + threadIdx.x; i < total; i += gridDim.x * blockDim.x) {
    const int k = i % Kpad;
    const int m = (i / Kpad) % Mpad;
    const int tap = i / (Kpad * Mpad);
    const int u = tap >> 1, v = tap & 1;
    __nv_bfloat16 val = __float2bfloat16(0.f);
    if (m < 4 * C && k < K) {
      const int cls = m / C, c = m % C;
      const int a = cls >> 1, b = cls & 1;
      const int r = a == 0 ? (u == 0 ? 1 : -1) : (u == 0 ? 2 : 0);
      const int sx = b == 0 ? (v == 0 ? 1 : -1) : (v == 0 ? 2 : 0);
      if (r >= 0 && sx >= 0) val = w[(((size_t)k * C + c) * 3 + r) * 3 + sx];
    }
    wp[i] = val;
  }
}
__global__ void interleave_s2_kernel(const __nv_bfloat16* __restrict__ t, __nv_bfloat16* __restrict__ dx, int N, int C,
                                     int Ho, int Wo) {
  const int wv = Wo / 8;
  const size_t total = (size_t)N * C * 2 * Ho * wv;
  for (size_t i = (size_t)blockIdx.x * blockDim.x + threadIdx.x; i < total; i += (size_t)gridDim.x * blockDim.x) {
    const int v = (int)(i % wv);
    const int oy = (int)((i / wv) % Ho);
    const int a = (int)((i / ((size_t)wv * Ho)) % 2);
    const size_t nc = i / ((size_t)wv * Ho * 2);
    const int c = (int)(nc % C);
    const size_t n = nc / C;
    const size_t plane = (size_t)Ho * Wo;
    const __nv_bfloat16* t0 = t + ((n * 4 + 2 * a) * C + c) * plane + (size_t)oy * Wo + v * 8;
    const uint4 e = __ldg(reinterpret_cast<const uint4*>(t0));
    const uint4 o = __ldg(reinterpret_cast<const uint4*>(t0 + (size_t)C * plane));
    uint4 lo, hi;
    lo.x = __byte_perm(e.x, o.x, 0x5410); lo.y = __byte_perm(e.x, o.x, 0x7632);
    lo.z = __byte_perm(e.y, o.y, 0x5410); lo.w = __byte_perm(e.y, o.y, 0x7632);
    hi.x = __byte_perm(e.z, o.z, 0x5410); hi.y = __byte_perm(e.z, o.z, 0x7632);
    hi.z = __byte_perm(e.w, o.w, 0x5410); hi.w = __byte_perm(e.w, o.w, 0x7632);
    uint4* d = reinterpret_cast<uint4*>(dx + ((nc * 2 * Ho) + 2 * oy + a) * (size_t)(2 * Wo) + v * 16);
    d[0] = lo; d[1] = hi;
  }
}

__global__ void subsample2_kernel(const __nv_bfloat16* __restrict__ x, __nv_bfloat16* __restrict__ y, size_t planes,
                                  int H, int W) {
  const int Ho = H / 2, Wo = W / 2, wv = Wo / 8;
  const size_t total = planes * Ho * wv;
  for (size_t i = (size_t)blockIdx.x * blockDim.x + threadIdx.x; i < total; i += (size_t)gridDim.x * blockDim.x) {
    const int v = (int)(i % wv);
    const int oy = (int)((i / wv) % Ho);
    const size_t pl = i / ((size_t)wv * Ho);
    const uint4* src = reinterpret_cast<const uint4*>(x + (pl * H + 2 * oy) * W + v * 16);
    const uint4 a = __ldg(src), b = __ldg(src + 1);
    uint4 o;
    o.x = __byte_perm(a.x, a.y, 0x5410);
    o.y = __byte_perm(a.z, a.w, 0x5410);
    o.z = __byte_perm(b.x, b.y, 0x5410);
    o.w = __byte_perm(b.z, b.w, 0x5410);
    *reinterpret_cast<uint4*>(y + (pl * Ho + oy) * Wo + v * 8) = o;
  }
}
__global__ void upsample2_zero_kernel(const __nv_bfloat16* __restrict__ g, __nv_bfloat16* __restrict__ dx,
                                      size_t planes, int H, int W) {
  const int Ho = H / 2, Wo = W / 2, wv = Wo / 8;
  const size_t total = planes * Ho * wv;
  const uint4 z = make_uint4(0, 0, 0, 0);
  for (size_t i = (size_t)blockIdx.x * blockDim.x + threadIdx.x; i < total; i += (size_t)gridDim.x * blockDim.x) {
    const int v = (int)(i % wv);
    const int oy = (int)((i / wv) % Ho);
    const size_t pl = i / ((size_t)wv * Ho);
    const uint4 a = __ldg(reinterpret_cast<const uint4*>(g + (pl * Ho + oy) * Wo + v * 8));
    uint4 lo, hi;
    lo.x = a.x & 0xFFFFu; lo.y = a.x >> 16; lo.z = a.y & 0xFFFFu; lo.w = a.y >> 16;
    hi.x = a.z & 0xFFFFu; hi.y = a.z >> 16; hi.z = a.w & 0xFFFFu; hi.w = a.w >> 16;
    uint4* d0 = reinterpret_cast<uint4*>(dx + (pl * H + 2 * oy) * W + v * 16);
    uint4* d1 = reinterpret_cast<uint4*>(dx + (pl * H + 2 * oy + 1) * W + v * 16);
    d0[0] = lo; d0[1] = hi; d1[0] = z; d1[1] = z;
  }
}
int launch_resample(bool up, const void* src, void* dst, size_t planes, int H, int W, cudaStream_t st) {
  const size_t total = planes * (H / 2) * (W / 16);
  size_t blocks = (total + 255) / 256;
  if (blocks > 148 * 32) blocks = 148 * 32;
  if (up)
    upsample2_zero_kernel<<<(int)blocks, 256, 0, st>>>((const __nv_bfloat16*)src, (__nv_bfloat16*)dst, planes, H, W);
  else
    subsample2_kernel<<<(int)blocks, 256, 0, st>>>((const __nv_bfloat16*)src, (__nv_bfloat16*)dst, planes, H, W);
  count_launch();
  SPC_CHECK_CUDA(cudaGetLastError());
  return SPC_OK;
}

__global__ void shift_copies_kernel(const __nv_bfloat16* __restrict__ x, __nv_bfloat16* __restrict__ xs,
                                    size_t planes, int H, int W, int S, int pw, int cs) {
  const int Wv = W / cs;
  const int wv = Wv / 8;
  const size_t rows = planes * H;
  const size_t total = rows * wv * S;
  for (size_t i = (size_t)blockIdx.x * blockDim.x + threadIdx.x; i < total; i += (size_t)gridDim.x * blockDim.x) {
    const int v = (int)(i % wv);
    const size_t row = (i / wv) % rows;
    const int sidx = (int)(i / ((size_t)wv * rows));
    const __nv_bfloat16* src = x + row * W;
    const int w0 = v * 8 * cs + sidx - pw;
    __nv_bfloat16 e[8];
#pragma unroll
    for (int j = 0; j < 8; ++j) {
      const int w = w0 + j * cs;
      e[j] = ((unsigned)w < (unsigned)W) ? src[w] : __float2bfloat16(0.f);
    }
    *reinterpret_cast<uint4*>(xs + ((size_t)sidx * rows + row) * Wv + v * 8) = *reinterpret_cast<const uint4*>(e);
  }
}
template <int S, int PW>
__global__ void __launch_bounds__(256)
shift_copies_vec_kernel(const __nv_bfloat16* __restrict__ x, __nv_bfloat16* __restrict__ xs, size_t planes, int H,
                        int W) {
  const int wv = W / 8;
  const size_t rows = planes * H;
  const size_t total = rows * wv;
  for (size_t i = (size_t)blockIdx.x * blockDim.x + threadIdx.x; i < total; i += (size_t)gridDim.x * blockDim.x) {
    const int v = (int)(i % wv);
    const size_t row = i / wv;
    const uint4* src = reinterpret_cast<const uint4*>(x + row * W) + v;
    const uint4 z = make_uint4(0, 0, 0, 0);
    const uint4 a = v > 0 ? __ldg(src - 1) : z;
    const uint4 b = __ldg(src);
    const uint4 c = v < wv - 1 ? __ldg(src + 1) : z;
    const uint32_t win[13] = {a.x, a.y, a.z, a.w, b.x, b.y, b.z, b.w, c.x, c.y, c.z, c.w, 0u};
#pragma unroll
    for (int sidx = 0; sidx < S; ++sidx) {
      const int e0 = 8 + sidx - PW;
      const int k = e0 >> 1;
      uint4 o;
      if (e0 & 1) {
        o.x = __funnelshift_r(win[k], win[k + 1], 16);
        o.y = __funnelshift_r(win[k + 1], win[k + 2], 16);
        o.z = __funnelshift_r(win[k + 2], win[k + 3], 16);
        o.w = __funnelshift_r(win[k + 3], win[k + 4], 16);
      } else {
        o.x = win[k]; o.y = win[k + 1]; o.z = win[k + 2]; o.w = win[k + 3];
      }
      *reinterpret_cast<uint4*>(xs + ((size_t)sidx * rows + row) * W + v * 8) = o;
    }
  }
}
__global__ void __launch_bounds__(256)
shift_copies_s2k3_kernel(const __nv_bfloat16* __restrict__ x, __nv_bfloat16* __restrict__ xs, size_t planes, int H,
                         int W) {
  const int Wv = W / 2, wv = Wv / 8;
  const size_t rows = planes * H;
  const size_t total = rows * wv;
  for (size_t i = (size_t)blockIdx.x * blockDim.x + threadIdx.x; i < total; i += (size_t)gridDim.x * blockDim.x) {
    const int v = (int)(i % wv);
    const size_t row = i / wv;
    const uint4* src = reinterpret_cast<const uint4*>(x + row * W) + 2 * v;
    const uint4 a = __ldg(src), b = __ldg(src + 1);
    const uint32_t prev = v > 0 ? (__ldg(reinterpret_cast<const uint32_t*>(src) - 1) >> 16) : 0u;
    uint4 ev, od, sh;
    ev.x = __byte_perm(a.x, a.y, 0x5410); ev.y = __byte_perm(a.z, a.w, 0x5410);
    ev.z = __byte_perm(b.x, b.y, 0x5410); ev.w = __byte_perm(b.z, b.w, 0x5410);
    od.x = __byte_perm(a.x, a.y, 0x7632); od.y = __byte_perm(a.z, a.w, 0x7632);
    od.z = __byte_perm(b.x, b.y, 0x7632); od.w = __byte_perm(b.z, b.w, 0x7632);
    sh.x = (od.x << 16) | prev;
    sh.y = __funnelshift_r(od.x, od.y, 16);
    sh.z = __funnelshift_r(od.y, od.z, 16);
    sh.w = __funnelshift_r(od.z, od.w, 16);
    __nv_bfloat16* dst = xs + row * Wv + v * 8;
    *reinterpret_cast<uint4*>(dst) = sh;
    *reinterpret_cast<uint4*>(dst + rows * Wv) = ev;
    *reinterpret_cast<uint4*>(dst + 2 * rows * Wv) = od;
  }
}
int launch_shift_copies(const void* x, void* xs, size_t planes, int H, int W, int S, int pw, int cs, cudaStream_t st) {
  const bool aligned = (reinterpret_cast<uintptr_t>(x) % 16 == 0) && (reinterpret_cast<uintptr_t>(xs) % 16 == 0);
  if (aligned && cs == 1 && W % 8 == 0 &&
      ((S == 7 && pw == 3) || (S == 3 && pw == 1) || (S == 5 && pw == 2) || (S == 2 && pw == 0))) {
    const size_t tot = planes * H * (W / 8);
    size_t blocks = (tot + 255) / 256;
    if (blocks > 148 * 32) blocks = 148 * 32;
    const __nv_bfloat16* xi = (const __nv_bfloat16*)x;
    __nv_bfloat16* xo = (__nv_bfloat16*)xs;
    if (S == 7) shift_copies_vec_kernel<7, 3><<<(int)blocks, 256, 0, st>>>(xi, xo, planes, H, W);
    else if (S == 3) shift_copies_vec_kernel<3, 1><<<(int)blocks, 256, 0, st>>>(xi, xo, planes, H, W);
    else if (S == 5) shift_copies_vec_kernel<5, 2><<<(int)blocks, 256, 0, st>>>(xi, xo, planes, H, W);
    else shift_copies_vec_kernel<2, 0><<<(int)blocks, 256, 0, st>>>(xi, xo, planes, H, W);
    count_launch();
    SPC_CHECK_CUDA(cudaGetLastError());
    return SPC_OK;
  }
  if (aligned && cs == 2 && S == 3 && pw == 1 && W % 16 == 0) {
    const size_t tot = planes * H * (W / 16);
    size_t blocks = (tot + 255) / 256;
    if (blocks > 148 * 32) blocks = 148 * 32;
    shift_copies_s2k3_kernel<<<(int)blocks, 256, 0, st>>>((const __nv_bfloat16*)x, (__nv_bfloat16*)xs, planes, H, W);
    count_launch();
    SPC_CHECK_CUDA(cudaGetLastError());
    return SPC_OK;
  }
  const size_t total = planes * H * (W / cs / 8) * S;
  size_t blocks = (total + 255) / 256;
  if (blocks > 148 * 32) blocks = 148 * 32;
  shift_copies_kernel<<<(int)blocks, 256, 0, st>>>((const __nv_bfloat16*)x, (__nv_bfloat16*)xs, planes, H, W, S, pw, cs);
  count_launch();
  SPC_CHECK_CUDA(cudaGetLastError());
  return SPC_OK;
}

inline bool is_s2(const spc_conv_desc* d) { return d->stride_h == 2 && d->stride_w == 2; }
inline size_t align1k(size_t b) { return (b + 1023) & ~(size_t)1023; }

bool tap_shape_ok(const spc_conv_desc* d) {
  if (d->dtype != SPC_BF16) return false;
  if (d->R * d->S == 1 || d->R * d->S > 49) return false;
  if ((d->R & 1) == 0 || (d->S & 1) == 0) return false;
  const bool s1 = d->stride_h == 1 && d->stride_w == 1, s2 = d->stride_h == 2 && d->stride_w == 2;
  if (!s1 && !s2) return false;
  if (s2 && (d->H % 2 || d->W % 2)) return false;
  const int Wo = d->W / d->stride_w;
  if (Wo % 64 != 0) return false;
  return (long long)d->H * d->W < (1ll << 31);
}

bool pw_shape_ok(const spc_conv_desc* d) {
  if (d->dtype != SPC_BF16) return false;
  if (d->R != 1 || d->S != 1) return false;
  long long P = (long long)d->H * d->W;
  if (is_s2(d)) {
    if (d->H % 2 || d->W % 32) return false;
    P /= 4;
  } else if (d->stride_h != 1 || d->stride_w != 1) {
    return false;
  }
  if (P % 8 != 0 || P >= (1ll << 31)) return false;
  return true;
}

}

bool tc_supported(const spc_conv_desc* d, int op) {
  if (pw_shape_ok(d)) return true;
  if (tap_shape_ok(d)) {
    if (tc_workspace_bytes(d, op) > (24ull << 30)) return false;
    if (op == 1 && is_s2(d)) return d->R == 3 && d->S == 3 && 4 * d->C <= 2048;
    return true;
  }
  return false;
}

static size_t wbytes(const spc_conv_desc* d, int op) {
  const size_t taps = (size_t)d->R * d->S;
  if (op == 0) return align1k(taps * round_up(d->K, 128) * round_up(d->C, BK) * 2 + 1024);
  if (op == 1) return align1k(taps * round_up(d->C, 128) * round_up(d->K, BK) * 2 + 1024);
  return 0;
}
size_t tc_workspace_bytes(const spc_conv_desc* d, int op) {
  const size_t taps = (size_t)d->R * d->S;
  const int cs = d->stride_w;
  size_t b = wbytes(d, op) + 4096;
  if (taps == 1) {
    if (is_s2(d)) b += align1k((size_t)d->N * d->C * (d->H / 2) * (d->W / 2) * 2) + 1024;
    return b;
  }
  const size_t Ho = d->H / cs, Wo = d->W / cs;
  if (op == 1 && is_s2(d)) {
    b = align1k(4ull * round_up(4 * d->C, 128) * round_up(d->K, BK) * 2) + 4096;
    b += align1k(2ull * d->N * d->K * Ho * Wo * 2) + align1k(4ull * d->N * d->C * Ho * Wo * 2) + 4096;
    return b;
  }
  if (op != 2 && !env_get("SPC_TAP_V1") &&
      tap_v2_supported(op == 1 ? d->C : d->K, op == 1 ? d->K : d->C, d->R, d->S, d->H, d->W, d->N, cs))
    return b;
  if (op == 2 && !env_get("SPC_TAP_V1") && wgrad_tap_supported(d->K, d->C, d->R, d->S, d->H, d->W, cs))
    return b;
  if (d->S > 1 || cs > 1)
    b += align1k((size_t)d->S * d->N * (op == 1 ? d->K : d->C) * d->H * Wo * 2) + 2048;
  return b;
}

int tc_conv_fwd(const spc_conv_desc* d, const void* x, const void* w, const void* bias, void* y, void* ws,
                size_t ws_bytes, cudaStream_t st) {
  SPC_REQUIRE(ws && ws_bytes >= tc_workspace_bytes(d, 0), "tcgen05 conv: workspace too small");
  if (d->R * d->S > 1) {
    TcConv c{};
    c.w = reinterpret_cast<const __nv_bfloat16*>(w);
    c.sm = (long long)d->C * d->R * d->S; c.sc = (long long)d->R * d->S; c.flip = 0;
    c.M = d->K; c.Cin = d->C; c.R = d->R; c.S = d->S; c.ph = d->pad_h; c.pw = d->pad_w;
    c.H = d->H; c.W = d->W; c.N = d->N; c.stride = d->stride_h;
    return run_conv_tc(c, reinterpret_cast<const __nv_bfloat16*>(x), reinterpret_cast<const __nv_bfloat16*>(bias),
                       reinterpret_cast<__nv_bfloat16*>(y), ws, ws_bytes, st);
  }
  if (is_s2(d)) {
    void* xs = reinterpret_cast<void*>(align1k(reinterpret_cast<uintptr_t>(ws) + wbytes(d, 0)));
    int rc = launch_resample(false, x, xs, (size_t)d->N * d->C, d->H, d->W, st);
    if (rc) return rc;
    return run_pw(reinterpret_cast<const __nv_bfloat16*>(w), d->C, 0, d->K, d->C,
                  reinterpret_cast<const __nv_bfloat16*>(xs), reinterpret_cast<const __nv_bfloat16*>(bias),
                  reinterpret_cast<__nv_bfloat16*>(y), d->N, (d->H / 2) * (d->W / 2), ws, wbytes(d, 0), st);
  }
  return run_pw(reinterpret_cast<const __nv_bfloat16*>(w), d->C, 0, d->K, d->C,
                reinterpret_cast<const __nv_bfloat16*>(x), reinterpret_cast<const __nv_bfloat16*>(bias),
                reinterpret_cast<__nv_bfloat16*>(y), d->N, d->H * d->W, ws, ws_bytes, st);
}

int tc_conv_dgrad(const spc_conv_desc* d, const void* dy, const void* w, void* dx, void* ws, size_t ws_bytes,
                  cudaStream_t st) {
  SPC_REQUIRE(ws && ws_bytes >= tc_workspace_bytes(d, 1), "tcgen05 conv: workspace too small");
  if (d->R * d->S > 1 && is_s2(d)) {
    const int Ho = d->H / 2, Wo = d->W / 2;
    const int Mq = 4 * d->C, Mpad = round_up(Mq, 128), Kpad = round_up(d->K, BK);
    uintptr_t a = align1k(reinterpret_cast<uintptr_t>(ws));
    __nv_bfloat16* wq = reinterpret_cast<__nv_bfloat16*>(a);
    a = align1k(a + (size_t)4 * Mpad * Kpad * 2);
    __nv_bfloat16* tmp = reinterpret_cast<__nv_bfloat16*>(a);
    a = align1k(a + (size_t)4 * d->N * d->C * Ho * Wo * 2);
    {
      const int total = 4 * Mpad * Kpad;
      int blocks = (total + 255) / 256;
      if (blocks > 1184) blocks = 1184;
      repack_dgrad_s2_kernel<<<blocks, 256, 0, st>>>(reinterpret_cast<const __nv_bfloat16*>(w), wq, d->K, d->C, Mpad, Kpad);
      count_launch();
      SPC_CHECK_CUDA(cudaGetLastError());
    }
    TcConv c{};
    c.prepacked = wq;
    c.M = Mq; c.Cin = d->K; c.R = 2; c.S = 2; c.ph = 0; c.pw = 0; c.H = Ho; c.W = Wo; c.N = d->N; c.stride = 1;
    int rc = run_conv_tc(c, reinterpret_cast<const __nv_bfloat16*>(dy), nullptr, tmp, reinterpret_cast<void*>(a),
                         ws_bytes - (a - reinterpret_cast<uintptr_t>(ws)), st);
    if (rc) return rc;
    const size_t total = (size_t)d->N * d->C * 2 * Ho * (Wo / 8);
    size_t blocks = (total + 255) / 256;
    if (blocks > 148 * 32) blocks = 148 * 32;
    interleave_s2_kernel<<<(int)blocks, 256, 0, st>>>(tmp, reinterpret_cast<__nv_bfloat16*>(dx), d->N, d->C, Ho, Wo);
    count_launch();
    SPC_CHECK_CUDA(cudaGetLastError());
    return SPC_OK;
  }
  if (d->R * d->S > 1) {
    TcConv c{};
    c.w = reinterpret_cast<const __nv_bfloat16*>(w);
    c.sm = (long long)d->R * d->S; c.sc = (long long)d->C * d->R * d->S; c.flip = 1;
    c.M = d->C; c.Cin = d->K; c.R = d->R; c.S = d->S; c.ph = d->R - 1 - d->pad_h; c.pw = d->S - 1 - d->pad_w;
    c.H = d->H; c.W = d->W; c.N = d->N; c.stride = 1;
    return run_conv_tc(c, reinterpret_cast<const __nv_bfloat16*>(dy), nullptr, reinterpret_cast<__nv_bfloat16*>(dx), ws,
                       ws_bytes, st);
  }
  if (is_s2(d)) {
    void* gs = reinterpret_cast<void*>(align1k(reinterpret_cast<uintptr_t>(ws) + wbytes(d, 1)));
    int rc = run_pw(reinterpret_cast<const __nv_bfloat16*>(w), d->C, 1, d->C, d->K,
                    reinterpret_cast<const __nv_bfloat16*>(dy), nullptr, reinterpret_cast<__nv_bfloat16*>(gs), d->N,
                    (d->H / 2) * (d->W / 2), ws, wbytes(d, 1), st);
    if (rc) return rc;
    return launch_resample(true, gs, dx, (size_t)d->N * d->C, d->H, d->W, st);
  }
  return run_pw(reinterpret_cast<const __nv_bfloat16*>(w), d->C, 1, d->C, d->K,
                reinterpret_cast<const __nv_bfloat16*>(dy), nullptr, reinterpret_cast<__nv_bfloat16*>(dx), d->N,
                d->H * d->W, ws, ws_bytes, st);
}

int tc_conv_wgrad(const spc_conv_desc* d, const void* x, const void* dy, float* dw, int accumulate, void* ws,
                  size_t ws_bytes, cudaStream_t st) {
  (void)accumulate;
  const __nv_bfloat16* xb = reinterpret_cast<const __nv_bfloat16*>(x);
  const __nv_bfloat16* dyb = reinterpret_cast<const __nv_bfloat16*>(dy);
  if (d->R * d->S > 1) {
    const int cs = d->stride_h;
    if (!env_get("SPC_TAP_V1") && wgrad_tap_supported(d->K, d->C, d->R, d->S, d->H, d->W, cs))
      return run_wgrad_tap(xb, dyb, dw, d->K, d->C, d->N, d->H, d->W, d->R, d->S, st);
    const bool copies = d->S > 1 || cs > 1;
    if (copies) {
      SPC_REQUIRE(ws && ws_bytes >= tc_workspace_bytes(d, 2), "tcgen05 wgrad: workspace too small");
      void* xs = reinterpret_cast<void*>(align1k(reinterpret_cast<uintptr_t>(ws)));
      int rc = launch_shift_copies(x, xs, (size_t)d->N * d->C, d->H, d->W, d->S, d->pad_w, cs, st);
      if (rc) return rc;
      xb = reinterpret_cast<const __nv_bfloat16*>(xs);
    }
    return run_wgrad(xb, dyb, dw, d->K, d->C, d->N, d->H / cs, d->W / cs, d->H, d->R, d->S, d->pad_h, cs, copies, st);
  }
  if (is_s2(d)) {
    SPC_REQUIRE(ws && ws_bytes >= tc_workspace_bytes(d, 2), "tcgen05 wgrad: workspace too small");
    void* xs = reinterpret_cast<void*>(align1k(reinterpret_cast<uintptr_t>(ws)));
    int rc = launch_resample(false, x, xs, (size_t)d->N * d->C, d->H, d->W, st);
    if (rc) return rc;
    return run_wgrad(reinterpret_cast<const __nv_bfloat16*>(xs), dyb, dw, d->K, d->C, d->N, 1, (d->H / 2) * (d->W / 2), 1,
                     1, 1, 0, 1, false, st);
  }
  return run_wgrad(xb, dyb, dw, d->K, d->C, d->N, 1, d->H * d->W, 1, 1, 1, 0, 1, false, st);
}

size_t tc_pw_workspace_bytes(int M, int Cin) { return (size_t)round_up(M, 128) * round_up(Cin, BK) * 2 + 4096; }
int tc_pw_fwd(const void* w, int ld, int M, int Cin, const void* x, const void* bias, void* y, int P, void* ws, size_t ws_bytes,
              cudaStream_t st) {
  return run_pw(reinterpret_cast<const __nv_bfloat16*>(w), ld, 0, M, Cin, reinterpret_cast<const __nv_bfloat16*>(x),
                reinterpret_cast<const __nv_bfloat16*>(bias), reinterpret_cast<__nv_bfloat16*>(y), 1, P, ws, ws_bytes, st);
}
int tc_pw_wgrad(const void* x, const void* dy, float* dw, int K, int C, int P, cudaStream_t st) {
  return run_wgrad(reinterpret_cast<const __nv_bfloat16*>(x), reinterpret_cast<const __nv_bfloat16*>(dy), dw, K, C, 1, 1, P, 1, 1, 1,
                   0, 1, false, st);
}

int make_tmap_ex(CUtensorMap* m, const void* base, int rank, const uint64_t* dims, const uint64_t* strides_bytes,
                 const uint32_t* box, int swizzle128) {
  return make_tmap_sw(m, base, rank, dims, strides_bytes, box,
                      swizzle128 ? CU_TENSOR_MAP_SWIZZLE_128B : CU_TENSOR_MAP_SWIZZLE_NONE);
}
int tc_sm_count() { return sm_count(); }

}

extern "C" void spc_reload_env(void) { spc::g_env_n = 0; }
```

mpi4dl_b200/csrc/wgrad_tap.cu:

```cuda
#include <stdlib.h>

#include "common.cuh"
#include "tc_common.cuh"

namespace spc {

using namespace tc;

int make_tmap_ex(CUtensorMap* m, const void* base, int rank, const uint64_t* dims, const uint64_t* strides_bytes,
                 const uint32_t* box, int swizzle128);
int tc_sm_count();

namespace {

constexpr int WT_THREADS = 448;
constexpr int SHIFT_THREADS = 256;
constexpr int RAW_ROW = 160;
constexpr int MAXP = 8;
constexpr int MAXRAW = 8;
constexpr int MAXQ = 16;

struct WtParams {
  float* dw;
  int K, C, R, S;
  int H, W, N;
  int modeB;
  int Pch, Qch, Qc16;
  int p_bytes;
  int p_blk;
  int qt_bytes;
  int ph, pw;
  int r0, nr, s0, ns;
  int rq;
  int psn, rawn;
  int nbw;
  int raw_bytes;
  int strips, row_splits, rows_per_split, num_items;
};

struct Ring {
  int i = 0;
  __device__ __forceinline__ int slot(int n) const { return i % n; }
  __device__ __forceinline__ int phase(int n) const { return (i / n) & 1; }
};

template <int D>
__device__ __forceinline__ uint4 shift_window(const uint32_t (&w)[8]) {
  static_assert(D >= -4 && D <= 4, "shift range");
  constexpr int e0 = 4 + D;
  constexpr int k = e0 >> 1;
  uint4 o;
  if (e0 & 1) {
    o.x = __funnelshift_r(w[k], w[k + 1], 16);
    o.y = __funnelshift_r(w[k + 1], w[k + 2], 16);
    o.z = __funnelshift_r(w[k + 2], w[k + 3], 16);
    o.w = __funnelshift_r(w[k + 3], w[k + 4], 16);
  } else {
    o.x = w[k]; o.y = w[k + 1]; o.z = w[k + 2]; o.w = w[k + 3];
  }
  return o;
}

template <int S, int SI>
struct ShiftCols {
  static __device__ __forceinline__ void run(const uint32_t (&win)[4][8], int qc16, int tid, uint8_t* dst, int qt_bytes, int s0,
                                             int ns) {
    if constexpr (SI < S) {
      if (SI >= s0 && SI < s0 + ns) {
        const int q = tid & 7, c0 = tid >> 3;
        uint8_t* t = dst + (SI - s0) * qt_bytes;
#pragma unroll
        for (int i = 0; i < 4; ++i) {
          const int c = c0 + 32 * i;
          if (c < qc16) *reinterpret_cast<uint4*>(t + c * 128 + ((q ^ (c & 7)) << 4)) = shift_window<SI - S / 2>(win[i]);
        }
      }
      ShiftCols<S, SI + 1>::run(win, qc16, tid, dst, qt_bytes, s0, ns);
    }
  }
};

template <int S>
__global__ void __launch_bounds__(WT_THREADS, 1)
wgrad_tap_kernel(const __grid_constant__ CUtensorMap tmap_p, const __grid_constant__ CUtensorMap tmap_q, const WtParams p) {
  constexpr bool SHIFT = S > 1;
  extern __shared__ uint8_t smem_raw[];
  uint8_t* smem = reinterpret_cast<uint8_t*>((reinterpret_cast<uintptr_t>(smem_raw) + 1023) & ~(uintptr_t)1023);
  const int qblk_bytes = p.ns * p.qt_bytes;
  const int qrow_bytes = p.nbw * qblk_bytes;
  const int prow_bytes = p.nbw * p.p_blk;
  const int rawrow_bytes = p.nbw * p.raw_bytes;
  uint8_t* p_base = smem;
  uint8_t* qt_base = p_base + p.psn * prow_bytes;
  uint8_t* raw_base = qt_base + p.rq * qrow_bytes;
  uint8_t* bar_base = raw_base + (SHIFT ? p.rawn * rawrow_bytes : 0);
  uint64_t* p_full = reinterpret_cast<uint64_t*>(bar_base);
  uint64_t* p_empty = p_full + MAXP;
  uint64_t* qt_full = p_empty + MAXP;
  uint64_t* qt_empty = qt_full + MAXQ;
  uint64_t* raw_full = qt_empty + MAXQ;
  uint64_t* raw_empty = raw_full + MAXRAW;
  uint64_t* tfull = raw_empty + MAXRAW;
  uint64_t* tempty = tfull + 1;
  uint32_t* tmem_slot = reinterpret_cast<uint32_t*>(tempty + 1);
  const int warp = threadIdx.x >> 5, lane = threadIdx.x & 31;

  if (threadIdx.x == 0) {
    for (int i = 0; i < MAXP; ++i) { mbar_init(&p_full[i], 1); mbar_init(&p_empty[i], 1); }
    for (int i = 0; i < MAXQ; ++i) { mbar_init(&qt_full[i], SHIFT ? SHIFT_THREADS : 1); mbar_init(&qt_empty[i], 1); }
    for (int i = 0; i < MAXRAW; ++i) { mbar_init(&raw_full[i], 1); mbar_init(&raw_empty[i], SHIFT_THREADS); }
    mbar_init(tfull, 1);
    mbar_init(tempty, 128);
    fence_barrier_init();
  }
  if (warp == 1) tmem_alloc(tmem_slot, 512);
  tc_fence_before();
  __syncthreads();
  tc_fence_after();
  const uint32_t tmem_base = *tmem_slot;

#define WT_ITEM(it)                                                               \
  const int sp_ = (it) % p.row_splits;                                            \
  const int strip_ = ((it) / p.row_splits) % p.strips;                            \
  const int n_ = (it) / (p.row_splits * p.strips);                                \
  const int w0 = strip_ * 64 * p.nbw;                                             \
  const int ha = sp_ * p.rows_per_split, hb = min(p.H, ha + p.rows_per_split);    \
  const int rows = hb - ha;                                                       \
  const int q_first = ha + p.r0 - p.ph;            \
  const int q_rows = rows + p.nr - 1;

  if (warp == 0) {
    if (lane == 0) {
      tma_prefetch_desc(&tmap_p);
      tma_prefetch_desc(&tmap_q);
      Ring qr, pr, rr;
      for (int it = blockIdx.x; it < p.num_items; it += gridDim.x) {
        WT_ITEM(it)
        if (rows <= 0) continue;
        for (int i = 0; i < q_rows; ++i) {
          if (SHIFT) {
            const int s = rr.slot(p.rawn);
            mbar_wait(&raw_empty[s], rr.phase(p.rawn) ^ 1);
            mbar_arrive_expect_tx(&raw_full[s], rawrow_bytes);
            for (int b = 0; b < p.nbw; ++b)
              tma_load_4d(raw_base + s * rawrow_bytes + b * p.raw_bytes, &tmap_q, &raw_full[s], w0 + 64 * b - 8, q_first + i, 0, n_);
            ++rr.i;
          } else {
            const int s = qr.slot(p.rq);
            mbar_wait(&qt_empty[s], qr.phase(p.rq) ^ 1);
            mbar_arrive_expect_tx(&qt_full[s], p.nbw * p.qt_bytes);
            for (int b = 0; b < p.nbw; ++b)
              tma_load_4d(qt_base + s * qrow_bytes + b * qblk_bytes, &tmap_q, &qt_full[s], w0 + 64 * b, q_first + i, 0, n_);
            ++qr.i;
          }
          if (i >= p.nr - 1) {
            const int j = i - (p.nr - 1);
            const int s = pr.slot(p.psn);
            mbar_wait(&p_empty[s], pr.phase(p.psn) ^ 1);
            mbar_arrive_expect_tx(&p_full[s], p.nbw * p.p_bytes);
            for (int b = 0; b < p.nbw; ++b)
              tma_load_4d(p_base + s * prow_bytes + b * p.p_blk, &tmap_p, &p_full[s], w0 + 64 * b, ha + j, 0, n_);
            ++pr.i;
          }
        }
      }
    }
  } else if (warp == 1) {
    if (lane == 0) {
      Ring qr, pr;
      int tph = 0;
      const int ngrp = (p.ns * p.Qc16 + 255) / 256;
      const int ns_g = (p.ns + ngrp - 1) / ngrp;
      for (int it = blockIdx.x; it < p.num_items; it += gridDim.x) {
        WT_ITEM(it)
        (void)w0; (void)n_; (void)q_first;
        if (rows <= 0) continue;
        mbar_wait(tempty, tph ^ 1);
        tc_fence_after();
        for (int j = 0; j < rows; ++j) {
          for (int i = (j == 0 ? 0 : p.nr - 1); i < p.nr; ++i) {
            const int g = qr.i + j + i;
            mbar_wait(&qt_full[g % p.rq], (g / p.rq) & 1);
          }
          const int ps = pr.slot(p.psn);
          mbar_wait(&p_full[ps], pr.phase(p.psn));
          tc_fence_after();
          for (int b = 0; b < p.nbw; ++b) {
            const uint32_t sa = smem_u32(p_base + ps * prow_bytes + b * p.p_blk);
            for (int r = 0; r < p.nr; ++r) {
              const int g = qr.i + j + r;
              const uint32_t sq = smem_u32(qt_base + (g % p.rq) * qrow_bytes + b * qblk_bytes);
              for (int sg = 0; sg * ns_g < p.ns; ++sg) {
                const int nsg = min(ns_g, p.ns - sg * ns_g);
                const uint32_t idesc = umma_idesc_bf16(128, nsg * p.Qc16, 0, 0);
                const uint32_t dcol = tmem_base + (uint32_t)((r * p.ns + sg * ns_g) * p.Qc16);
#pragma unroll
                for (int ks = 0; ks < 4; ++ks) {
                  const uint64_t adesc = umma_desc(sa + ks * 32, 16, 1024);
                  const uint64_t bdesc = umma_desc(sq + sg * ns_g * p.qt_bytes + ks * 32, 16, 1024);
                  umma_bf16(dcol, adesc, bdesc, idesc, (j | b | ks) ? 1u : 0u);
                }
              }
            }
          }
          umma_commit(&p_empty[ps]);
          ++pr.i;
          { const int g = qr.i + j; umma_commit(&qt_empty[g % p.rq]); }
        }
        for (int i = rows; i < q_rows; ++i) { const int g = qr.i + i; umma_commit(&qt_empty[g % p.rq]); }
        qr.i += q_rows;
        umma_commit(tfull);
        tph ^= 1;
      }
    }
  } else if (warp >= 6) {
    if (SHIFT) {
      const int tid = threadIdx.x - 6 * 32;
      const int q = tid & 7, c0 = tid >> 3;
      Ring qr, rr;
      for (int it = blockIdx.x; it < p.num_items; it += gridDim.x) {
        WT_ITEM(it)
        (void)w0; (void)n_; (void)q_first;
        if (rows <= 0) continue;
        for (int i = 0; i < q_rows; ++i) {
          const int rs = rr.slot(p.rawn);
          mbar_wait(&raw_full[rs], rr.phase(p.rawn));
          const int qs = qr.slot(p.rq);
          for (int b = 0; b < p.nbw; ++b) {
            const uint8_t* raw = raw_base + rs * rawrow_bytes + b * p.raw_bytes;
            uint32_t win[4][8];
#pragma unroll
            for (int k = 0; k < 4; ++k) {
              const int c = c0 + 32 * k;
              if (c < p.Qc16) {
                const uint8_t* row = raw + c * RAW_ROW;
                const uint4 own = *reinterpret_cast<const uint4*>(row + 16 * (q + 1));
                uint32_t lz = __shfl_up_sync(0xffffffffu, own.z, 1), lw = __shfl_up_sync(0xffffffffu, own.w, 1);
                uint32_t rx = __shfl_down_sync(0xffffffffu, own.x, 1), ry = __shfl_down_sync(0xffffffffu, own.y, 1);
                if (q == 0) { const uint2 h = *reinterpret_cast<const uint2*>(row + 8); lz = h.x; lw = h.y; }
                if (q == 7) { const uint2 h = *reinterpret_cast<const uint2*>(row + 16 * 9); rx = h.x; ry = h.y; }
                win[k][0] = lz; win[k][1] = lw; win[k][2] = own.x; win[k][3] = own.y;
                win[k][4] = own.z; win[k][5] = own.w; win[k][6] = rx; win[k][7] = ry;
              }
            }
            if (b == p.nbw - 1) mbar_arrive(&raw_empty[rs]);
            if (b == 0) mbar_wait(&qt_empty[qs], qr.phase(p.rq) ^ 1);
            ShiftCols<S, 0>::run(win, p.Qc16, tid, qt_base + qs * qrow_bytes + b * qblk_bytes, p.qt_bytes, p.s0, p.ns);
          }
          ++rr.i;
          fence_proxy_async();
          mbar_arrive(&qt_full[qs]);
          ++qr.i;
        }
      }
    }
  } else if (warp >= 2 && warp <= 5) {
    const int quarter = warp & 3;
    const int pl = quarter * 32 + lane;
    int tph = 0;
    for (int it = blockIdx.x; it < p.num_items; it += gridDim.x) {
      WT_ITEM(it)
      (void)w0; (void)n_; (void)q_first; (void)q_rows;
      if (rows <= 0) continue;
      mbar_wait(tfull, tph);
      tc_fence_after();
      const int ncols = p.nr * p.ns * p.Qc16;
#pragma unroll 1
      for (int c32 = 0; c32 < ncols; c32 += 32) {
        uint32_t v[32];
        tmem_ld_32x32(tmem_base + ((uint32_t)(quarter * 32) << 16) + c32, v);
        tmem_ld_wait();
        if (pl < p.Pch) {
#pragma unroll
          for (int e = 0; e < 32; ++e) {
            const int col = c32 + e;
            if (col < ncols) {
              const int tap = col / p.Qc16, qc = col - tap * p.Qc16;
              if (qc < p.Qch) {
                int r = p.r0 + tap / p.ns, s = p.s0 + tap % p.ns;
                int k, c;
                if (p.modeB) { k = qc; c = pl; r = p.R - 1 - r; s = p.S - 1 - s; } else { k = pl; c = qc; }
                atomicAdd(&p.dw[(((size_t)k * p.C + c) * p.R + r) * p.S + s], __uint_as_float(v[e]));
              }
            }
          }
        }
      }
      tc_fence_before();
      mbar_arrive(tempty);
      tph ^= 1;
    }
  }
#undef WT_ITEM
  tc_fence_before();
  __syncthreads();
  if (warp == 1) tmem_dealloc(tmem_base, 512);
}

constexpr int WT_SMEM_LIMIT = 222 * 1024;
constexpr int WT_SMEM_AUX = 1024 + 1024;
inline int rup(int a, int b) { return (a + b - 1) / b * b; }

template <int S>
int launch_wt(const CUtensorMap& tp, const CUtensorMap& tq, const WtParams& p, int smem, cudaStream_t st) {
  auto kern = wgrad_tap_kernel<S>;
  static bool attr_set = false;
  if (!attr_set) {
    SPC_CHECK_CUDA(cudaFuncSetAttribute(kern, cudaFuncAttributeMaxDynamicSharedMemorySize, WT_SMEM_LIMIT));
    attr_set = true;
  }
  const int sms = tc_sm_count();
  kern<<<p.num_items < sms ? p.num_items : sms, WT_THREADS, smem, st>>>(tp, tq, p);
  count_launch();
  SPC_CHECK_CUDA(cudaGetLastError());
  return SPC_OK;
}

int plan_passes(int R, int S, int Qc16, int (*rect)[4]) {
  const int maxt = 512 / Qc16;
  if (maxt < 1) return 0;
  int n = 0;
  if (R * S <= maxt) { rect[n][0] = 0; rect[n][1] = R; rect[n][2] = 0; rect[n][3] = S; return 1; }
  if (S <= maxt) {
    const int nr = maxt / S;
    for (int r0 = 0; r0 < R; r0 += nr, ++n) { rect[n][0] = r0; rect[n][1] = min(nr, R - r0); rect[n][2] = 0; rect[n][3] = S; }
    return n;
  }
  if (R == 1) {
    const int np = (S + maxt - 1) / maxt, per = (S + np - 1) / np;
    for (int s0 = 0; s0 < S; s0 += per, ++n) { rect[n][0] = 0; rect[n][1] = 1; rect[n][2] = s0; rect[n][3] = min(per, S - s0); }
    return n;
  }
  return 0;
}

}

bool wgrad_tap_supported(int K, int C, int R, int S, int H, int W, int stride) {
  if (stride != 1 || R * S == 1 || (W % 64) != 0 || H < 1) return false;
  if (!(S == 3 || S == 5 || S == 7) || (R & 1) == 0 || R > 7) return false;
  if (K > 128 || C > 128) return false;
  const int Qc16 = rup(K >= C ? C : K, 16);
  int rect[16][4];
  return plan_passes(R, S, Qc16, rect) > 0;
}

int run_wgrad_tap(const __nv_bfloat16* x, const __nv_bfloat16* dy, float* dw, int K, int C, int N, int H, int W, int R, int S,
                  cudaStream_t st) {
  WtParams p{};
  p.dw = dw; p.K = K; p.C = C; p.R = R; p.S = S; p.H = H; p.W = W; p.N = N;
  p.ph = (R - 1) / 2; p.pw = (S - 1) / 2;
  p.modeB = K >= C ? 0 : 1;
  p.Pch = p.modeB ? C : K; p.Qch = p.modeB ? K : C;
  p.Qc16 = rup(p.Qch, 16);
  p.p_bytes = rup(p.Pch, 8) * 128;
  p.p_blk = rup(p.p_bytes, 1024);
  p.qt_bytes = p.Qc16 * 128;
  p.raw_bytes = p.Qc16 * RAW_ROW;
  const __nv_bfloat16* P = p.modeB ? x : dy;
  const __nv_bfloat16* Q = p.modeB ? dy : x;
  int rect[16][4];
  const int npass = plan_passes(R, S, p.Qc16, rect);
  SPC_REQUIRE(npass > 0, "wgrad_tap: %dx%d filter with %d Q channels does not fit TMEM", R, S, p.Qch);
  CUtensorMap tp, tq;
  {
    const uint64_t dims[4] = {(uint64_t)W, (uint64_t)H, (uint64_t)p.Pch, (uint64_t)N};
    const uint64_t strides[4] = {0, (uint64_t)W * 2, (uint64_t)H * W * 2, (uint64_t)H * W * p.Pch * 2};
    const uint32_t box[4] = {64, 1, (uint32_t)rup(p.Pch, 8), 1};
    int rc = make_tmap_ex(&tp, P, 4, dims, strides, box, 1);
    if (rc) return rc;
  }
  {
    const uint64_t dims[4] = {(uint64_t)W, (uint64_t)H, (uint64_t)p.Qch, (uint64_t)N};
    const uint64_t strides[4] = {0, (uint64_t)W * 2, (uint64_t)H * W * 2, (uint64_t)H * W * p.Qch * 2};
    const uint32_t box[4] = {(uint32_t)(S > 1 ? 80 : 64), 1, (uint32_t)p.Qc16, 1};
    int rc = make_tmap_ex(&tq, Q, 4, dims, strides, box, S > 1 ? 0 : 1);
    if (rc) return rc;
  }
  const int sms = tc_sm_count();
  p.nbw = 1;
  {
    const int rowb = rup(p.Pch, 8) * 128 + p.Qc16 * 128;
    while (p.nbw < 4 && rowb * p.nbw < 12 * 1024 && W % (128 * p.nbw) == 0) p.nbw *= 2;
  }
  p.strips = W / (64 * p.nbw);
  for (int pi = 0; pi < npass; ++pi) {
    p.r0 = rect[pi][0]; p.nr = rect[pi][1]; p.s0 = rect[pi][2]; p.ns = rect[pi][3];
    const int qrow_bytes = p.nbw * p.ns * p.qt_bytes, prow = p.nbw * p.p_blk, rawrow = S > 1 ? p.nbw * p.raw_bytes : 0;
    const bool small_rows = prow + p.nbw * p.qt_bytes < 12 * 1024;
    p.psn = 3; p.rawn = S > 1 ? 2 : 0; p.rq = p.nr + 1;
    int rem = WT_SMEM_LIMIT - WT_SMEM_AUX - p.psn * prow - p.rawn * rawrow - p.rq * qrow_bytes;
    SPC_REQUIRE(rem >= 0, "wgrad_tap: shared memory too small (rows %d, %d bytes per row)", p.nr, qrow_bytes);
    if (small_rows) {
      for (bool grew = true; grew;) {
        grew = false;
        if (S > 1 && p.rawn < MAXRAW && rem >= rawrow) { ++p.rawn; rem -= rawrow; grew = true; }
        if (p.psn < MAXP && rem >= prow) { ++p.psn; rem -= prow; grew = true; }
        if (p.rq < MAXQ && p.rq < p.nr + 8 && rem >= qrow_bytes) { ++p.rq; rem -= qrow_bytes; grew = true; }
      }
    } else {
      while (p.rq < p.nr + 3 && p.rq < MAXQ && rem >= qrow_bytes) { ++p.rq; rem -= qrow_bytes; }
    }
    const int base_items = N * p.strips;
    int best = 1;
    double best_eff = 0.0;
    for (int sp = 1; sp <= 64 && H / sp >= 8 * p.nr; ++sp) {
      const int items = base_items * sp, waves = (items + sms - 1) / sms;
      if (waves > 3) break;
      const double eff = (double)items / ((double)waves * sms) * (1.0 - (double)(p.nr - 1) * sp / (H + (p.nr - 1) * sp));
      if (eff > best_eff + 1e-9) { best_eff = eff; best = sp; }
    }
    p.row_splits = best;
    p.rows_per_split = (H + best - 1) / best;
    p.num_items = base_items * best;
    const int smem = p.psn * prow + p.rq * qrow_bytes + p.rawn * rawrow + WT_SMEM_AUX;
    int rc;
    if (S == 1) rc = launch_wt<1>(tp, tq, p, smem, st);
    else if (S == 3) rc = launch_wt<3>(tp, tq, p, smem, st);
    else if (S == 5) rc = launch_wt<5>(tp, tq, p, smem, st);
    else if (S == 7) rc = launch_wt<7>(tp, tq, p, smem, st);
    else { set_error("wgrad_tap: unsupported filter width %d", S); return SPC_EUNSUPPORTED; }
    if (rc) return rc;
  }
  return SPC_OK;
}

}
```

Before: 5.961.

## Add stride-2 3x3 support to tap conv and wgrad kernels with in-smem deinterleave

```diff
diff --git a/mpi4dl_b200/csrc/conv_tap.cu b/mpi4dl_b200/csrc/conv_tap.cu
--- a/mpi4dl_b200/csrc/conv_tap.cu
+++ b/mpi4dl_b200/csrc/conv_tap.cu
@@ -16,11 +16,13 @@
 constexpr int TAP_THREADS = 448;
 constexpr int BLK = 8192;
 constexpr int RAW_SHIFT_ROW = 160;
+constexpr int RAW_S2_ROW = 272;
 constexpr int MAXRING = 8;
 constexpr int STAGE_BYTES = 128 * 128;
 
 struct TapParams {
   int M, Cin, H, W, N;
+  int Ho;
   int R, ph;
   int Mpad;
   int mrows;
@@ -34,6 +36,7 @@
   int opblk;
   int group;
   int rows_raw;
+  int nstage;
   int dbg;
   const __nv_bfloat16* bias;
   __nv_bfloat16* y;
@@ -109,10 +112,57 @@
   }
 };
 
-template <int NB, int S>
+template <int NB>
+struct ShiftRowS2 {
+  static __device__ __forceinline__ void run(const uint8_t* rawr, int row_step, int cv, int tid, uint8_t* op_base, int opblk,
+                                             int group, uint64_t* op_full, uint64_t* op_empty, RingState& ro, int ops) {
+    const int q = tid & 7, c0 = tid >> 3;
+    uint4 t[2 * NB][3];
+#pragma unroll
+    for (int i = 0; i < 2 * NB; ++i) {
+      const int j = i >> 1, c = c0 + 32 * (i & 1);
+      if (c < cv) {
+        const uint8_t* row = rawr + j * row_step + c * RAW_S2_ROW;
+        const uint4 a = *reinterpret_cast<const uint4*>(row + 16 + 32 * q);
+        const uint4 b = *reinterpret_cast<const uint4*>(row + 32 + 32 * q);
+        uint32_t prev = __shfl_up_sync(0xffffffffu, b.w, 1) >> 16;
+        if (q == 0) prev = *reinterpret_cast<const uint16_t*>(row + 14);
+        uint4 ev, od, sh;
+        ev.x = __byte_perm(a.x, a.y, 0x5410); ev.y = __byte_perm(a.z, a.w, 0x5410);
+        ev.z = __byte_perm(b.x, b.y, 0x5410); ev.w = __byte_perm(b.z, b.w, 0x5410);
+        od.x = __byte_perm(a.x, a.y, 0x7632); od.y = __byte_perm(a.z, a.w, 0x7632);
+        od.z = __byte_perm(b.x, b.y, 0x7632); od.w = __byte_perm(b.z, b.w, 0x7632);
+        sh.x = (od.x << 16) | prev;
+        sh.y = __funnelshift_r(od.x, od.y, 16);
+        sh.z = __funnelshift_r(od.y, od.z, 16);
+        sh.w = __funnelshift_r(od.z, od.w, 16);
+        t[i][0] = sh; t[i][1] = ev; t[i][2] = od;
+      }
+    }
+    const int tile_bytes = NB * opblk;
+#pragma unroll
+    for (int si = 0; si < 3; ++si) {
+      if (!group || si == 0) mbar_wait(&op_empty[ro.s], ro.ph ^ 1);
+      uint8_t* opb = op_base + ro.s * (group ? 3 : 1) * tile_bytes + (group ? si * tile_bytes : 0);
+#pragma unroll
+      for (int i = 0; i < 2 * NB; ++i) {
+        const int j = i >> 1, c = c0 + 32 * (i & 1);
+        if (c < cv) *reinterpret_cast<uint4*>(opb + j * opblk + c * 128 + ((q ^ (c & 7)) << 4)) = t[i][si];
+      }
+      if (!group || si == 2) {
+        fence_proxy_async();
+        mbar_arrive(&op_full[ro.s]);
+        ro.next(ops);
+      }
+    }
+  }
+};
+
+template <int NB, int S, int CS>
 __global__ void __launch_bounds__(TAP_THREADS, 1)
 conv_tap_kernel(const __grid_constant__ CUtensorMap tmap_w, const __grid_constant__ CUtensorMap tmap_x,
                 const __grid_constant__ CUtensorMap tmap_y, const TapParams p) {
+  static_assert(CS == 1 || S == 3, "stride 2: 3 filter columns only");
   constexpr bool SHIFT = S > 1;
   constexpr int NPIX = NB * 64;
   const int RAW_BLK = p.raw_blk;
@@ -125,7 +175,7 @@
   uint8_t* op_base = raw_base + p.rawb * p.rows_raw * RAW_BLK;
   const int slot_bytes = (p.group ? S : 1) * NB * p.opblk;
   uint8_t* stage_base = op_base + (SHIFT ? p.ops * slot_bytes : 0);
-  uint8_t* bar_base = stage_base + STAGE_BYTES;
+  uint8_t* bar_base = stage_base + p.nstage * STAGE_BYTES;
   uint64_t* raw_full = reinterpret_cast<uint64_t*>(bar_base);
   uint64_t* raw_empty = raw_full + MAXRING;
   uint64_t* a_full = raw_empty + MAXRING;
@@ -184,7 +234,8 @@
         mbar_wait(&raw_empty[rb.s], rb.ph ^ 1);
         mbar_arrive_expect_tx(&raw_full[rb.s], p.rows_raw * RAW_BLK);
         for (int i = 0; i < p.rows_raw; ++i)
-          tma_load_4d(raw_base + (rb.s * p.rows_raw + i) * RAW_BLK, &tmap_x, &raw_full[rb.s], w0 - xoff, h0 - p.ph + i, 0, n_);
+          tma_load_4d(raw_base + (rb.s * p.rows_raw + i) * RAW_BLK, &tmap_x, &raw_full[rb.s], CS * w0 - xoff, CS * h0 - p.ph + i, 0,
+                      n_);
         rb.next(p.rawb);
       }
       while (ct < p.num_tiles) {
@@ -210,7 +261,7 @@
             if (armed) {
               const int quota = ((tap + 1) * p.rows_raw + taps - 1) / taps;
               for (; row < quota; ++row)
-                tma_load_4d(dst + row * RAW_BLK, &tmap_x, &raw_full[rb.s], w0 - xoff, h0 - p.ph + row, nkc * 64, n_);
+                tma_load_4d(dst + row * RAW_BLK, &tmap_x, &raw_full[rb.s], CS * w0 - xoff, CS * h0 - p.ph + row, nkc * 64, n_);
             }
           }
         }
@@ -220,7 +271,7 @@
             mbar_arrive_expect_tx(&raw_full[rb.s], p.rows_raw * RAW_BLK);
           }
           for (; row < p.rows_raw; ++row)
-            tma_load_4d(dst + row * RAW_BLK, &tmap_x, &raw_full[rb.s], w0 - xoff, h0 - p.ph + row, nkc * 64, n_);
+            tma_load_4d(dst + row * RAW_BLK, &tmap_x, &raw_full[rb.s], CS * w0 - xoff, CS * h0 - p.ph + row, nkc * 64, n_);
           rb.next(p.rawb);
         }
         ct = nt; ckc = nkc;
@@ -278,8 +329,12 @@
           if (!(p.dbg & 2)) mbar_wait(&raw_full[rb.s], rb.ph);
           const int cv = (p.dbg & 8) ? 0 : min(64, (p.Cin - kc * 64 + 15) & ~15);
           const uint8_t* rawb = raw_base + rb.s * p.rows_raw * RAW_BLK;
-          for (int r = 0; r < p.R; ++r)
-            ShiftRow<NB, S, 0>::run(rawb + r * RAW_BLK, RAW_BLK, cv, tid, op_base, p.opblk, p.group, op_full, op_empty, ro, p.ops);
+          for (int r = 0; r < p.R; ++r) {
+            if constexpr (CS == 2)
+              ShiftRowS2<NB>::run(rawb + r * RAW_BLK, 2 * RAW_BLK, cv, tid, op_base, p.opblk, p.group, op_full, op_empty, ro, p.ops);
+            else
+              ShiftRow<NB, S, 0>::run(rawb + r * RAW_BLK, RAW_BLK, cv, tid, op_base, p.opblk, p.group, op_full, op_empty, ro, p.ops);
+          }
           if (!(p.dbg & 2)) mbar_arrive(&raw_empty[rb.s]);
           rb.next(p.rawb);
         }
@@ -291,20 +346,25 @@
     const float bias = (k < p.M && p.bias) ? __bfloat162float(p.bias[k]) : 0.f;
     const bool leader = threadIdx.x == 64;
     int acc = 0, aph = 0;
+    int sb = 0;
     for (int t = blockIdx.x; t < p.num_tiles; t += gridDim.x) {
       TAP_TILE_DECODE(t)
       mbar_wait(&tfull[acc], aph);
       tc_fence_after();
 #pragma unroll 1
       for (int j = 0; j < NB; ++j) {
-        if (leader) tma_store_wait_read<0>();
+        if (leader) {
+          if (p.nstage == 2) tma_store_wait_read<1>();
+          else tma_store_wait_read<0>();
+        }
+        uint8_t* stage = stage_base + sb * STAGE_BYTES;
         named_bar_sync(1, 128);
 #pragma unroll
         for (int cc = 0; cc < 2; ++cc) {
           uint32_t r[32];
           tmem_ld_32x32(tmem_base + ((uint32_t)(quarter * 32) << 16) + acc * NPIX + j * 64 + cc * 32, r);
           tmem_ld_wait();
-          uint8_t* rowp = stage_base + k * 128;
+          uint8_t* rowp = stage + k * 128;
 #pragma unroll
           for (int v = 0; v < 4; ++v) {
             uint4 o;
@@ -322,9 +382,12 @@
         }
         fence_proxy_async();
         named_bar_sync(1, 128);
-        if (leader && !(p.dbg & 4) && h0 + j < p.H) {
-          tma_store_4d(&tmap_y, stage_base, w0, h0 + j, 0, n_);
-          tma_store_commit();
+        if (!(p.dbg & 4) && h0 + j < p.Ho) {
+          if (leader) {
+            tma_store_4d(&tmap_y, stage, w0, h0 + j, 0, n_);
+            tma_store_commit();
+          }
+          if (p.nstage == 2) sb ^= 1;
         }
       }
       if (++acc == 2) { acc = 0; aph ^= 1; }
@@ -348,23 +411,25 @@
   int smem;
 };
 
-bool plan_tap(int M, int Cin, int R, int S, int H, int W, int N, TapPlan* out) {
+bool plan_tap(int M, int Cin, int R, int S, int H, int W, int N, int cs, TapPlan* out) {
   TapParams p{};
   p.M = M; p.Cin = Cin; p.H = H; p.W = W; p.N = N; p.R = R;
+  p.Ho = H / cs;
   p.mrows = round_up_i(M, 8);
   p.a_blk = round_up_i(p.mrows * 128, 1024);
   p.kchunks = (Cin + 63) / 64;
   const int taps = R * S;
   const bool shift = S > 1;
   p.cbox = Cin >= 64 ? 64 : round_up_i(Cin, 16);
-  p.raw_blk = p.cbox * (shift ? RAW_SHIFT_ROW : 128);
+  p.raw_blk = p.cbox * (cs == 2 ? RAW_S2_ROW : shift ? RAW_SHIFT_ROW : 128);
   const int raw_blk = p.raw_blk;
   const int budget = TAP_SMEM_LIMIT - TAP_SMEM_AUX;
   p.opblk = p.cbox * 128;
   const int budget_ops = budget - STAGE_BYTES;
-  for (int NB = 4; NB >= 2; NB -= 2) {
-    if (NB == 4 && H < 4) continue;
-    p.rows_raw = NB + R - 1;
+  const int nb_hi = cs == 2 ? 2 : 4;
+  for (int NB = nb_hi; NB >= nb_hi / 2; NB /= 2) {
+    if (NB == nb_hi && p.Ho < nb_hi) continue;
+    p.rows_raw = cs * (NB - 1) + R;
     const int raw_buf = p.rows_raw * raw_blk;
     const int a_res = taps * p.kchunks * p.a_blk;
     for (int resident = 1; resident >= 0; --resident) {
@@ -376,13 +441,15 @@
         int rem = budget_ops - a_bytes - rawb * raw_buf - ops * slot;
         if (rem < 0) continue;
         if (shift && !group && rem >= slot) { ++ops; rem -= slot; }
+        p.nstage = 1;
+        if (cs == 2 && rem >= STAGE_BYTES && !getenv("SPC_X_NSTAGE1")) { p.nstage = 2; rem -= STAGE_BYTES; }
         while (!resident && ast < MAXRING && rem >= p.a_blk) { ++ast; rem -= p.a_blk; }
         while (rawb < 4 && rem >= raw_buf) { ++rawb; rem -= raw_buf; }
         while (shift && ops < 4 && rem >= slot) { ++ops; rem -= slot; }
         a_bytes = resident ? a_res : ast * p.a_blk;
         p.a_resident = resident; p.ast = ast; p.ops = ops; p.rawb = rawb; p.group = group;
         out->NB = NB; out->p = p;
-        out->smem = a_bytes + rawb * raw_buf + ops * slot + STAGE_BYTES + TAP_SMEM_AUX;
+        out->smem = a_bytes + rawb * raw_buf + ops * slot + p.nstage * STAGE_BYTES + TAP_SMEM_AUX;
         return true;
       }
     }
@@ -390,10 +457,10 @@
   return false;
 }
 
-template <int NB, int S>
+template <int NB, int S, int CS>
 int launch_tap(const CUtensorMap& tw, const CUtensorMap& tx, const CUtensorMap& ty, const TapParams& p, int smem,
                cudaStream_t st) {
-  auto kern = conv_tap_kernel<NB, S>;
+  auto kern = conv_tap_kernel<NB, S, CS>;
   static bool attr_set = false;
   if (!attr_set) {
     SPC_CHECK_CUDA(cudaFuncSetAttribute(kern, cudaFuncAttributeMaxDynamicSharedMemorySize, TAP_SMEM_LIMIT));
@@ -410,24 +477,32 @@
 }
 
 bool tap_v2_supported(int M, int Cin, int R, int S, int H, int W, int N, int stride) {
-  if (stride != 1 || M > 128 || R * S == 1 || (W % 64) != 0 || H < 2) return false;
-  if (!(S == 1 || S == 3 || S == 5 || S == 7) || (R & 1) == 0 || R > 7) return false;
+  if (M > 128 || R * S == 1) return false;
+  if (stride == 2) {
+    if (R != 3 || S != 3 || H % 2 || W % 2 || (W / 2) % 64 != 0 || H < 2) return false;
+    if (Cin > 16 && !getenv("SPC_X_S2ALL_F")) return false;
+  } else {
+    if (stride != 1 || (W % 64) != 0 || H < 2) return false;
+    if (!(S == 1 || S == 3 || S == 5 || S == 7) || (R & 1) == 0 || R > 7) return false;
+  }
   TapPlan pl;
-  return plan_tap(M, Cin, R, S, H, W, N, &pl);
+  return plan_tap(M, Cin, R, S, H, W, N, stride, &pl);
 }
 
 int run_conv_tap_v2(const __nv_bfloat16* wp, int Mpad, int Cpad, const __nv_bfloat16* x, const __nv_bfloat16* bias,
-                    __nv_bfloat16* y, int M, int Cin, int R, int S, int ph, int H, int W, int N, cudaStream_t st) {
+                    __nv_bfloat16* y, int M, int Cin, int R, int S, int ph, int H, int W, int N, int cs, cudaStream_t st) {
   TapPlan pl;
-  SPC_REQUIRE(plan_tap(M, Cin, R, S, H, W, N, &pl), "tap conv: no shared-memory plan for M=%d Cin=%d %dx%d", M, Cin, R, S);
+  SPC_REQUIRE(plan_tap(M, Cin, R, S, H, W, N, cs, &pl), "tap conv: no shared-memory plan for M=%d Cin=%d %dx%d stride %d", M,
+              Cin, R, S, cs);
   TapParams& p = pl.p;
   p.ph = ph; p.Mpad = Mpad; p.bias = bias; p.y = y;
   {
     const char* e = getenv("SPC_TAP_DBG");
     p.dbg = e ? atoi(e) : 0;
   }
-  p.tiles_w = W / 64;
-  p.tiles_h = (H + pl.NB - 1) / pl.NB;
+  const int Wo = W / cs;
+  p.tiles_w = Wo / 64;
+  p.tiles_h = (p.Ho + pl.NB - 1) / pl.NB;
   p.num_tiles = p.tiles_w * p.tiles_h * N;
   CUtensorMap tw, tx, ty;
   {
@@ -440,19 +515,20 @@
   {
     const uint64_t dims[4] = {(uint64_t)W, (uint64_t)H, (uint64_t)Cin, (uint64_t)N};
     const uint64_t strides[4] = {0, (uint64_t)W * 2, (uint64_t)H * W * 2, (uint64_t)H * W * Cin * 2};
-    const uint32_t box[4] = {(uint32_t)(S > 1 ? 80 : 64), 1, (uint32_t)p.cbox, 1};
+    const uint32_t box[4] = {(uint32_t)(cs == 2 ? 136 : S > 1 ? 80 : 64), 1, (uint32_t)p.cbox, 1};
     int rc = make_tmap_ex(&tx, x, 4, dims, strides, box, S > 1 ? 0 : 1);
     if (rc) return rc;
   }
   {
-    const uint64_t dims[4] = {(uint64_t)W, (uint64_t)H, (uint64_t)M, (uint64_t)N};
-    const uint64_t strides[4] = {0, (uint64_t)W * 2, (uint64_t)H * W * 2, (uint64_t)H * W * M * 2};
+    const uint64_t dims[4] = {(uint64_t)Wo, (uint64_t)p.Ho, (uint64_t)M, (uint64_t)N};
+    const uint64_t strides[4] = {0, (uint64_t)Wo * 2, (uint64_t)p.Ho * Wo * 2, (uint64_t)p.Ho * Wo * M * 2};
     const uint32_t box[4] = {64, 1, 128, 1};
     int rc = make_tmap_ex(&ty, y, 4, dims, strides, box, 1);
     if (rc) return rc;
   }
-#define TAP_CASE(nb, s) if (pl.NB == nb && S == s) return launch_tap<nb, s>(tw, tx, ty, p, pl.smem, st);
-  TAP_CASE(2, 1) TAP_CASE(4, 1) TAP_CASE(2, 3) TAP_CASE(4, 3) TAP_CASE(2, 5) TAP_CASE(4, 5) TAP_CASE(2, 7) TAP_CASE(4, 7)
+#define TAP_CASE(nb, s, c) if (pl.NB == nb && S == s && cs == c) return launch_tap<nb, s, c>(tw, tx, ty, p, pl.smem, st);
+  TAP_CASE(2, 1, 1) TAP_CASE(4, 1, 1) TAP_CASE(2, 3, 1) TAP_CASE(4, 3, 1) TAP_CASE(2, 5, 1) TAP_CASE(4, 5, 1) TAP_CASE(2, 7, 1)
+  TAP_CASE(4, 7, 1) TAP_CASE(1, 3, 2) TAP_CASE(2, 3, 2)
 #undef TAP_CASE
   set_error("tap conv: unsupported filter width %d", S);
   return SPC_EUNSUPPORTED;
diff --git a/mpi4dl_b200/csrc/gemm_tc.cu b/mpi4dl_b200/csrc/gemm_tc.cu
--- a/mpi4dl_b200/csrc/gemm_tc.cu
+++ b/mpi4dl_b200/csrc/gemm_tc.cu
@@ -9,11 +9,11 @@
 
 bool tap_v2_supported(int M, int Cin, int R, int S, int H, int W, int N, int stride);
 int run_conv_tap_v2(const __nv_bfloat16* wp, int Mpad, int Cpad, const __nv_bfloat16* x, const __nv_bfloat16* bias,
-                    __nv_bfloat16* y, int M, int Cin, int R, int S, int ph, int H, int W, int N, cudaStream_t st);
+                    __nv_bfloat16* y, int M, int Cin, int R, int S, int ph, int H, int W, int N, int cs, cudaStream_t st);
 
 bool wgrad_tap_supported(int K, int C, int R, int S, int H, int W, int stride);
 int run_wgrad_tap(const __nv_bfloat16* x, const __nv_bfloat16* dy, float* dw, int K, int C, int N, int H, int W, int R, int S,
-                  cudaStream_t st);
+                  int cs, cudaStream_t st);
 
 namespace {
 
@@ -371,6 +371,12 @@
   const int v = e ? atoi(e) : 0;
   return v > 0 ? v : dflt;
 }
+
+inline bool tap_kernels_on(int stride) {
+  if (env_get("SPC_TAP_V1")) return false;
+  const char* s2 = env_get("SPC_TAP_S2");
+  return stride == 1 || !(s2 && atoi(s2) == 0);
+}
 inline int sm_count() {
   static int sms = 0;
   if (!sms) {
@@ -460,7 +466,7 @@
   const int Ho = c.H / cs, Wo = c.W / cs;
   const int Pin = c.H * c.W, P = Ho * Wo;
   const int Mpad = round_up(c.M, 128), Cpad = round_up(c.Cin, BK);
-  const bool v2 = taps > 1 && !env_get("SPC_TAP_V1") && tap_v2_supported(c.M, c.Cin, c.R, c.S, c.H, c.W, c.N, cs);
+  const bool v2 = taps > 1 && tap_kernels_on(cs) && tap_v2_supported(c.M, c.Cin, c.R, c.S, c.H, c.W, c.N, cs);
   const bool copies = (c.S > 1 || cs > 1) && taps > 1 && !v2;
   const uintptr_t ws0 = reinterpret_cast<uintptr_t>(ws);
   const uintptr_t wp_addr = (ws0 + 1023) & ~(uintptr_t)1023;
@@ -481,7 +487,7 @@
     wp = wpm;
   }
   if (v2)
-    return run_conv_tap_v2(wp, Mpad, Cpad, x, bias, y, c.M, c.Cin, c.R, c.S, c.ph, c.H, c.W, c.N, st);
+    return run_conv_tap_v2(wp, Mpad, Cpad, x, bias, y, c.M, c.Cin, c.R, c.S, c.ph, c.H, c.W, c.N, cs, st);
   const __nv_bfloat16* xsrc = x;
   if (copies) {
     void* xs = reinterpret_cast<void*>(xs_addr);
@@ -1386,10 +1392,10 @@
     b += align1k(2ull * d->N * d->K * Ho * Wo * 2) + align1k(4ull * d->N * d->C * Ho * Wo * 2) + 4096;
     return b;
   }
-  if (op != 2 && !env_get("SPC_TAP_V1") &&
+  if (op != 2 && tap_kernels_on(cs) &&
       tap_v2_supported(op == 1 ? d->C : d->K, op == 1 ? d->K : d->C, d->R, d->S, d->H, d->W, d->N, cs))
     return b;
-  if (op == 2 && !env_get("SPC_TAP_V1") && wgrad_tap_supported(d->K, d->C, d->R, d->S, d->H, d->W, cs))
+  if (op == 2 && tap_kernels_on(cs) && wgrad_tap_supported(d->K, d->C, d->R, d->S, d->H, d->W, cs))
     return b;
   if (d->S > 1 || cs > 1)
     b += align1k((size_t)d->S * d->N * (op == 1 ? d->K : d->C) * d->H * Wo * 2) + 2048;
@@ -1483,8 +1489,8 @@
   const __nv_bfloat16* dyb = reinterpret_cast<const __nv_bfloat16*>(dy);
   if (d->R * d->S > 1) {
     const int cs = d->stride_h;
-    if (!env_get("SPC_TAP_V1") && wgrad_tap_supported(d->K, d->C, d->R, d->S, d->H, d->W, cs))
-      return run_wgrad_tap(xb, dyb, dw, d->K, d->C, d->N, d->H, d->W, d->R, d->S, st);
+    if (tap_kernels_on(cs) && wgrad_tap_supported(d->K, d->C, d->R, d->S, d->H, d->W, cs))
+      return run_wgrad_tap(xb, dyb, dw, d->K, d->C, d->N, d->H, d->W, d->R, d->S, cs, st);
     const bool copies = d->S > 1 || cs > 1;
     if (copies) {
       SPC_REQUIRE(ws && ws_bytes >= tc_workspace_bytes(d, 2), "tcgen05 wgrad: workspace too small");
diff --git a/mpi4dl_b200/csrc/wgrad_tap.cu b/mpi4dl_b200/csrc/wgrad_tap.cu
--- a/mpi4dl_b200/csrc/wgrad_tap.cu
+++ b/mpi4dl_b200/csrc/wgrad_tap.cu
@@ -16,6 +16,7 @@
 constexpr int WT_THREADS = 448;
 constexpr int SHIFT_THREADS = 256;
 constexpr int RAW_ROW = 160;
+constexpr int RAW_S2_ROW = 272;
 constexpr int MAXP = 8;
 constexpr int MAXRAW = 8;
 constexpr int MAXQ = 16;
@@ -32,6 +33,7 @@
   int ph, pw;
   int r0, nr, s0, ns;
   int rq;
+  int adv, qstep;
   int psn, rawn;
   int nbw;
   int raw_bytes;
@@ -61,6 +63,23 @@
   return o;
 }
 
+__device__ __forceinline__ void deinterleave_s2(const uint8_t* row, int q, uint4 (&t)[3]) {
+  const uint4 a = *reinterpret_cast<const uint4*>(row + 16 + 32 * q);
+  const uint4 b = *reinterpret_cast<const uint4*>(row + 32 + 32 * q);
+  uint32_t prev = __shfl_up_sync(0xffffffffu, b.w, 1) >> 16;
+  if (q == 0) prev = *reinterpret_cast<const uint16_t*>(row + 14);
+  uint4 ev, od, sh;
+  ev.x = __byte_perm(a.x, a.y, 0x5410); ev.y = __byte_perm(a.z, a.w, 0x5410);
+  ev.z = __byte_perm(b.x, b.y, 0x5410); ev.w = __byte_perm(b.z, b.w, 0x5410);
+  od.x = __byte_perm(a.x, a.y, 0x7632); od.y = __byte_perm(a.z, a.w, 0x7632);
+  od.z = __byte_perm(b.x, b.y, 0x7632); od.w = __byte_perm(b.z, b.w, 0x7632);
+  sh.x = (od.x << 16) | prev;
+  sh.y = __funnelshift_r(od.x, od.y, 16);
+  sh.z = __funnelshift_r(od.y, od.z, 16);
+  sh.w = __funnelshift_r(od.z, od.w, 16);
+  t[0] = sh; t[1] = ev; t[2] = od;
+}
+
 template <int S, int SI>
 struct ShiftCols {
   static __device__ __forceinline__ void run(const uint32_t (&win)[4][8], int qc16, int tid, uint8_t* dst, int qt_bytes, int s0,
@@ -80,10 +99,12 @@
   }
 };
 
-template <int S>
+template <int S, int CS>
 __global__ void __launch_bounds__(WT_THREADS, 1)
 wgrad_tap_kernel(const __grid_constant__ CUtensorMap tmap_p, const __grid_constant__ CUtensorMap tmap_q, const WtParams p) {
+  static_assert(CS == 1 || S == 3, "stride 2: 3 filter columns only");
   constexpr bool SHIFT = S > 1;
+  const int adv = CS == 1 ? 1 : p.adv, qstep = CS == 1 ? 1 : p.qstep;
   extern __shared__ uint8_t smem_raw[];
   uint8_t* smem = reinterpret_cast<uint8_t*>((reinterpret_cast<uintptr_t>(smem_raw) + 1023) & ~(uintptr_t)1023);
   const int qblk_bytes = p.ns * p.qt_bytes;
@@ -126,8 +147,8 @@
   const int w0 = strip_ * 64 * p.nbw;                                             \
   const int ha = sp_ * p.rows_per_split, hb = min(p.H, ha + p.rows_per_split);    \
   const int rows = hb - ha;                                                       \
-  const int q_first = ha + p.r0 - p.ph;            \
-  const int q_rows = rows + p.nr - 1;
+  const int q_first = CS * ha + p.r0 - p.ph;       \
+  const int q_rows = adv * (rows - 1) + p.nr;
 
   if (warp == 0) {
     if (lane == 0) {
@@ -143,7 +164,8 @@
             mbar_wait(&raw_empty[s], rr.phase(p.rawn) ^ 1);
             mbar_arrive_expect_tx(&raw_full[s], rawrow_bytes);
             for (int b = 0; b < p.nbw; ++b)
-              tma_load_4d(raw_base + s * rawrow_bytes + b * p.raw_bytes, &tmap_q, &raw_full[s], w0 + 64 * b - 8, q_first + i, 0, n_);
+              tma_load_4d(raw_base + s * rawrow_bytes + b * p.raw_bytes, &tmap_q, &raw_full[s], CS * (w0 + 64 * b) - 8,
+                          q_first + qstep * i, 0, n_);
             ++rr.i;
           } else {
             const int s = qr.slot(p.rq);
@@ -153,8 +175,8 @@
               tma_load_4d(qt_base + s * qrow_bytes + b * qblk_bytes, &tmap_q, &qt_full[s], w0 + 64 * b, q_first + i, 0, n_);
             ++qr.i;
           }
-          if (i >= p.nr - 1) {
-            const int j = i - (p.nr - 1);
+          if (i >= p.nr - 1 && (i - (p.nr - 1)) % adv == 0) {
+            const int j = (i - (p.nr - 1)) / adv;
             const int s = pr.slot(p.psn);
             mbar_wait(&p_empty[s], pr.phase(p.psn) ^ 1);
             mbar_arrive_expect_tx(&p_full[s], p.nbw * p.p_bytes);
@@ -178,8 +200,8 @@
         mbar_wait(tempty, tph ^ 1);
         tc_fence_after();
         for (int j = 0; j < rows; ++j) {
-          for (int i = (j == 0 ? 0 : p.nr - 1); i < p.nr; ++i) {
-            const int g = qr.i + j + i;
+          for (int i = (j == 0 ? 0 : adv * (j - 1) + p.nr); i < adv * j + p.nr; ++i) {
+            const int g = qr.i + i;
             mbar_wait(&qt_full[g % p.rq], (g / p.rq) & 1);
           }
           const int ps = pr.slot(p.psn);
@@ -188,7 +210,7 @@
           for (int b = 0; b < p.nbw; ++b) {
             const uint32_t sa = smem_u32(p_base + ps * prow_bytes + b * p.p_blk);
             for (int r = 0; r < p.nr; ++r) {
-              const int g = qr.i + j + r;
+              const int g = qr.i + adv * j + r;
               const uint32_t sq = smem_u32(qt_base + (g % p.rq) * qrow_bytes + b * qblk_bytes);
               for (int sg = 0; sg * ns_g < p.ns; ++sg) {
                 const int nsg = min(ns_g, p.ns - sg * ns_g);
@@ -205,9 +227,12 @@
           }
           umma_commit(&p_empty[ps]);
           ++pr.i;
-          { const int g = qr.i + j; umma_commit(&qt_empty[g % p.rq]); }
+          for (int i = adv * j; i < adv * (j + 1); ++i) {
+            const int g = qr.i + i;
+            umma_commit(&qt_empty[g % p.rq]);
+          }
         }
-        for (int i = rows; i < q_rows; ++i) { const int g = qr.i + i; umma_commit(&qt_empty[g % p.rq]); }
+        for (int i = adv * rows; i < q_rows; ++i) { const int g = qr.i + i; umma_commit(&qt_empty[g % p.rq]); }
         qr.i += q_rows;
         umma_commit(tfull);
         tph ^= 1;
@@ -228,24 +253,46 @@
           const int qs = qr.slot(p.rq);
           for (int b = 0; b < p.nbw; ++b) {
             const uint8_t* raw = raw_base + rs * rawrow_bytes + b * p.raw_bytes;
-            uint32_t win[4][8];
-#pragma unroll
-            for (int k = 0; k < 4; ++k) {
-              const int c = c0 + 32 * k;
-              if (c < p.Qc16) {
-                const uint8_t* row = raw + c * RAW_ROW;
-                const uint4 own = *reinterpret_cast<const uint4*>(row + 16 * (q + 1));
-                uint32_t lz = __shfl_up_sync(0xffffffffu, own.z, 1), lw = __shfl_up_sync(0xffffffffu, own.w, 1);
-                uint32_t rx = __shfl_down_sync(0xffffffffu, own.x, 1), ry = __shfl_down_sync(0xffffffffu, own.y, 1);
-                if (q == 0) { const uint2 h = *reinterpret_cast<const uint2*>(row + 8); lz = h.x; lw = h.y; }
-                if (q == 7) { const uint2 h = *reinterpret_cast<const uint2*>(row + 16 * 9); rx = h.x; ry = h.y; }
-                win[k][0] = lz; win[k][1] = lw; win[k][2] = own.x; win[k][3] = own.y;
-                win[k][4] = own.z; win[k][5] = own.w; win[k][6] = rx; win[k][7] = ry;
+            if constexpr (CS == 2) {
+              uint4 t[4][3];
+#pragma unroll
+              for (int k = 0; k < 4; ++k) {
+                const int c = c0 + 32 * k;
+                if (c < p.Qc16) deinterleave_s2(raw + c * RAW_S2_ROW, q, t[k]);
               }
+              if (b == p.nbw - 1) mbar_arrive(&raw_empty[rs]);
+              if (b == 0) mbar_wait(&qt_empty[qs], qr.phase(p.rq) ^ 1);
+              uint8_t* dst = qt_base + qs * qrow_bytes + b * qblk_bytes;
+#pragma unroll
+              for (int si = 0; si < 3; ++si) {
+                if (si < p.s0 || si >= p.s0 + p.ns) continue;
+#pragma unroll
+                for (int k = 0; k < 4; ++k) {
+                  const int c = c0 + 32 * k;
+                  if (c < p.Qc16)
+                    *reinterpret_cast<uint4*>(dst + (si - p.s0) * p.qt_bytes + c * 128 + ((q ^ (c & 7)) << 4)) = t[k][si];
+                }
+              }
+            } else {
+              uint32_t win[4][8];
+#pragma unroll
+              for (int k = 0; k < 4; ++k) {
+                const int c = c0 + 32 * k;
+                if (c < p.Qc16) {
+                  const uint8_t* row = raw + c * RAW_ROW;
+                  const uint4 own = *reinterpret_cast<const uint4*>(row + 16 * (q + 1));
+                  uint32_t lz = __shfl_up_sync(0xffffffffu, own.z, 1), lw = __shfl_up_sync(0xffffffffu, own.w, 1);
+                  uint32_t rx = __shfl_down_sync(0xffffffffu, own.x, 1), ry = __shfl_down_sync(0xffffffffu, own.y, 1);
+                  if (q == 0) { const uint2 h = *reinterpret_cast<const uint2*>(row + 8); lz = h.x; lw = h.y; }
+                  if (q == 7) { const uint2 h = *reinterpret_cast<const uint2*>(row + 16 * 9); rx = h.x; ry = h.y; }
+                  win[k][0] = lz; win[k][1] = lw; win[k][2] = own.x; win[k][3] = own.y;
+                  win[k][4] = own.z; win[k][5] = own.w; win[k][6] = rx; win[k][7] = ry;
+                }
+              }
+              if (b == p.nbw - 1) mbar_arrive(&raw_empty[rs]);
+              if (b == 0) mbar_wait(&qt_empty[qs], qr.phase(p.rq) ^ 1);
+              ShiftCols<S, 0>::run(win, p.Qc16, tid, qt_base + qs * qrow_bytes + b * qblk_bytes, p.qt_bytes, p.s0, p.ns);
             }
-            if (b == p.nbw - 1) mbar_arrive(&raw_empty[rs]);
-            if (b == 0) mbar_wait(&qt_empty[qs], qr.phase(p.rq) ^ 1);
-            ShiftCols<S, 0>::run(win, p.Qc16, tid, qt_base + qs * qrow_bytes + b * qblk_bytes, p.qt_bytes, p.s0, p.ns);
           }
           ++rr.i;
           fence_proxy_async();
@@ -301,9 +348,9 @@
 constexpr int WT_SMEM_AUX = 1024 + 1024;
 inline int rup(int a, int b) { return (a + b - 1) / b * b; }
 
-template <int S>
+template <int S, int CS>
 int launch_wt(const CUtensorMap& tp, const CUtensorMap& tq, const WtParams& p, int smem, cudaStream_t st) {
-  auto kern = wgrad_tap_kernel<S>;
+  auto kern = wgrad_tap_kernel<S, CS>;
   static bool attr_set = false;
   if (!attr_set) {
     SPC_CHECK_CUDA(cudaFuncSetAttribute(kern, cudaFuncAttributeMaxDynamicSharedMemorySize, WT_SMEM_LIMIT));
@@ -337,6 +384,12 @@
 }
 
 bool wgrad_tap_supported(int K, int C, int R, int S, int H, int W, int stride) {
+  if (stride == 2) {
+    if (R != 3 || S != 3 || H % 2 || W % 2 || (W / 2) % 64 != 0 || K > 128 || C > 128) return false;
+    if ((C <= 16 || C > 64) && !getenv("SPC_X_S2ALL_W")) return false;
+    int rect[16][4];
+    return plan_passes(R, S, rup(C, 16), rect) > 0;
+  }
   if (stride != 1 || R * S == 1 || (W % 64) != 0 || H < 1) return false;
   if (!(S == 3 || S == 5 || S == 7) || (R & 1) == 0 || R > 7) return false;
   if (K > 128 || C > 128) return false;
@@ -346,17 +399,19 @@
 }
 
 int run_wgrad_tap(const __nv_bfloat16* x, const __nv_bfloat16* dy, float* dw, int K, int C, int N, int H, int W, int R, int S,
-                  cudaStream_t st) {
+                  int cs, cudaStream_t st) {
   WtParams p{};
+  const int Hi = H, Wi = W;
+  H /= cs; W /= cs;
   p.dw = dw; p.K = K; p.C = C; p.R = R; p.S = S; p.H = H; p.W = W; p.N = N;
   p.ph = (R - 1) / 2; p.pw = (S - 1) / 2;
-  p.modeB = K >= C ? 0 : 1;
+  p.modeB = (cs == 1 && K < C) ? 1 : 0;
   p.Pch = p.modeB ? C : K; p.Qch = p.modeB ? K : C;
   p.Qc16 = rup(p.Qch, 16);
   p.p_bytes = rup(p.Pch, 8) * 128;
   p.p_blk = rup(p.p_bytes, 1024);
   p.qt_bytes = p.Qc16 * 128;
-  p.raw_bytes = p.Qc16 * RAW_ROW;
+  p.raw_bytes = p.Qc16 * (cs == 2 ? RAW_S2_ROW : RAW_ROW);
   const __nv_bfloat16* P = p.modeB ? x : dy;
   const __nv_bfloat16* Q = p.modeB ? dy : x;
   int rect[16][4];
@@ -371,9 +426,9 @@
     if (rc) return rc;
   }
   {
-    const uint64_t dims[4] = {(uint64_t)W, (uint64_t)H, (uint64_t)p.Qch, (uint64_t)N};
-    const uint64_t strides[4] = {0, (uint64_t)W * 2, (uint64_t)H * W * 2, (uint64_t)H * W * p.Qch * 2};
-    const uint32_t box[4] = {(uint32_t)(S > 1 ? 80 : 64), 1, (uint32_t)p.Qc16, 1};
+    const uint64_t dims[4] = {(uint64_t)Wi, (uint64_t)Hi, (uint64_t)p.Qch, (uint64_t)N};
+    const uint64_t strides[4] = {0, (uint64_t)Wi * 2, (uint64_t)Hi * Wi * 2, (uint64_t)Hi * Wi * p.Qch * 2};
+    const uint32_t box[4] = {(uint32_t)(cs == 2 ? 136 : S > 1 ? 80 : 64), 1, (uint32_t)p.Qc16, 1};
     int rc = make_tmap_ex(&tq, Q, 4, dims, strides, box, S > 1 ? 0 : 1);
     if (rc) return rc;
   }
@@ -386,9 +441,11 @@
   p.strips = W / (64 * p.nbw);
   for (int pi = 0; pi < npass; ++pi) {
     p.r0 = rect[pi][0]; p.nr = rect[pi][1]; p.s0 = rect[pi][2]; p.ns = rect[pi][3];
+    p.adv = (cs == 2 && p.nr > 1) ? 2 : 1;
+    p.qstep = (cs == 2 && p.nr == 1) ? 2 : 1;
     const int qrow_bytes = p.nbw * p.ns * p.qt_bytes, prow = p.nbw * p.p_blk, rawrow = S > 1 ? p.nbw * p.raw_bytes : 0;
-    const bool small_rows = prow + p.nbw * p.qt_bytes < 12 * 1024;
-    p.psn = 3; p.rawn = S > 1 ? 2 : 0; p.rq = p.nr + 1;
+    const bool small_rows = prow + p.nbw * p.qt_bytes < 12 * 1024 || (cs == 2 && !getenv("SPC_X_WTGROW0"));
+    p.psn = 3; p.rawn = S > 1 ? 2 : 0; p.rq = p.nr + p.adv;
     int rem = WT_SMEM_LIMIT - WT_SMEM_AUX - p.psn * prow - p.rawn * rawrow - p.rq * qrow_bytes;
     SPC_REQUIRE(rem >= 0, "wgrad_tap: shared memory too small (rows %d, %d bytes per row)", p.nr, qrow_bytes);
     if (small_rows) {
@@ -396,10 +453,10 @@
         grew = false;
         if (S > 1 && p.rawn < MAXRAW && rem >= rawrow) { ++p.rawn; rem -= rawrow; grew = true; }
         if (p.psn < MAXP && rem >= prow) { ++p.psn; rem -= prow; grew = true; }
-        if (p.rq < MAXQ && p.rq < p.nr + 8 && rem >= qrow_bytes) { ++p.rq; rem -= qrow_bytes; grew = true; }
+        if (p.rq < MAXQ && p.rq < p.nr + 8 * p.adv && rem >= qrow_bytes) { ++p.rq; rem -= qrow_bytes; grew = true; }
       }
     } else {
-      while (p.rq < p.nr + 3 && p.rq < MAXQ && rem >= qrow_bytes) { ++p.rq; rem -= qrow_bytes; }
+      while (p.rq < p.nr + 3 * p.adv && p.rq < MAXQ && rem >= qrow_bytes) { ++p.rq; rem -= qrow_bytes; }
     }
     const int base_items = N * p.strips;
     int best = 1;
@@ -415,10 +472,12 @@
     p.num_items = base_items * best;
     const int smem = p.psn * prow + p.rq * qrow_bytes + p.rawn * rawrow + WT_SMEM_AUX;
     int rc;
-    if (S == 1) rc = launch_wt<1>(tp, tq, p, smem, st);
-    else if (S == 3) rc = launch_wt<3>(tp, tq, p, smem, st);
-    else if (S == 5) rc = launch_wt<5>(tp, tq, p, smem, st);
-    else if (S == 7) rc = launch_wt<7>(tp, tq, p, smem, st);
+    if (cs == 2 && S == 3) rc = launch_wt<3, 2>(tp, tq, p, smem, st);
+    else if (cs != 1) { set_error("wgrad_tap: unsupported stride %d", cs); return SPC_EUNSUPPORTED; }
+    else if (S == 1) rc = launch_wt<1, 1>(tp, tq, p, smem, st);
+    else if (S == 3) rc = launch_wt<3, 1>(tp, tq, p, smem, st);
+    else if (S == 5) rc = launch_wt<5, 1>(tp, tq, p, smem, st);
+    else if (S == 7) rc = launch_wt<7, 1>(tp, tq, p, smem, st);
     else { set_error("wgrad_tap: unsupported filter width %d", S); return SPC_EUNSUPPORTED; }
     if (rc) return rc;
   }
```

Measured after the change: 6.016 (median of 6 runs). No clear change (+0.9%).
